# labicon/dp-ilqr

Measured on AMD Instinct MI355X. Metric: ilqr_subproblems_per_sec, higher is better.
Workload: dtype f64; 1 GPU; cfg2: batches of 1024 independent 5-agent DoubleIntDynamics4D iLQR sub-problems per GPU per step, T=50, scripts/analysis.py scenario distribution, tol=1e-3, n_lqr_iter=50; 2468 steps = 2527232 distinct seeds per GPU, window of 6144 in flight; 1 repetition(s) of the job on disjoint seeds, the median is reported; batch_per_gpu=1024, window=6144, n_x=20, n_u=10, horizon=50, parallelism=single GPU

## Files before the change

### dpilqr_amd/csrc/admit_order.hpp

```cpp
#pragma once
#include <cstdint>

#if defined(__HIPCC__)
#include <hip/hip_runtime.h>
#define DPILQR_HD __host__ __device__
#else
#define DPILQR_HD
#endif

namespace dpilqr {

enum CostOrder : int { kOrderOff = 0, kOrderSpread = 1, kOrderGrouped = 2 };
constexpr int kDefaultCostOrder = kOrderSpread;

constexpr int kOrderMinLive = 1024;
constexpr int kOrderClasses = 64;

struct SweepDeal {
    int n, n_cus, waves, per_layer, layers, rounds, lo, extra;
    DPILQR_HD SweepDeal(int n_, int n_cus_, int waves_) : n(n_), n_cus(n_cus_), waves(waves_) {
        const int lpr = waves / 4;
        per_layer = 4 * n_cus;
        layers = (n + per_layer - 1) / per_layer;
        rounds = (layers + lpr - 1) / lpr;
        lo = rounds > 0 ? layers / rounds : 0;
        extra = rounds > 0 ? layers - lo * rounds : 0;
    }
    DPILQR_HD int layers_of(int round) const { return lo + (round < extra ? 1 : 0); }
    DPILQR_HD int first_layer(int round) const { return round * lo + (round < extra ? round : extra); }
    DPILQR_HD int round_of_layer(int layer) const {
        const int head = extra * (lo + 1);
        return layer < head ? layer / (lo + 1) : extra + (layer - head) / (lo > 0 ? lo : 1);
    }
    DPILQR_HD int slot(int round, int cu, int wave) const {
        if (round >= rounds || wave >= 4 * layers_of(round)) return -1;
        const int s = (first_layer(round) + (wave >> 2)) * per_layer + (wave & 3) * n_cus + cu;
        return s < n ? s : -1;
    }
};

DPILQR_HD inline int order_position(int rank, const SweepDeal& D, int order) {
    if (order != kOrderGrouped) return rank;
    const int round = D.round_of_layer(rank / D.per_layer);
    const int f = D.first_layer(round), m = D.layers_of(round);
    const int q = rank - f * D.per_layer;
    int base = 4 * m, e = 0;
    if (round == D.rounds - 1) {
        const int rem = D.n - (D.layers - 1) * D.per_layer;
        base = 4 * (m - 1) + rem / D.n_cus;
        e = rem % D.n_cus;
    }
    int cu, w;
    if (q < e * (base + 1)) { cu = q / (base + 1); w = q - cu * (base + 1); }
    else { const int q2 = q - e * (base + 1), per = base > 0 ? base : 1; cu = e + q2 / per; w = q2 - (cu - e) * per; }
    return (f + (w >> 2)) * D.per_layer + (w & 3) * D.n_cus + cu;
}

DPILQR_HD inline int order_class(int key, int T) {
    const int top = T + 1;
    const int c = top < kOrderClasses ? key : (int)((int64_t)key * (kOrderClasses - 1) / top);
    return c < 0 ? 0 : (c > kOrderClasses - 1 ? kOrderClasses - 1 : c);
}

#if defined(__HIPCC__) && defined(DPILQR_ADMIT_ORDER_KERNELS)

constexpr int kKeyStagedAgents = 5;
__global__ void __launch_bounds__(256) k_cost_keys(const double* __restrict__ X, const double* __restrict__ radius, int64_t radius_bstride,
                                                   const int32_t* __restrict__ list, const int32_t* __restrict__ count, int B, int T, int k,
                                                   int min_live, int32_t* __restrict__ key) {
    __shared__ double2 sP[4][64 * kKeyStagedAgents];
    const int n = count ? *count : B;
    if (n <= min_live) return;
    const int wave = (int)threadIdx.x >> 6, lane = threadIdx.x & 63;
    const int pos = (int)blockIdx.x * 4 + wave;
    if (pos >= n) return;
    const int b = list ? list[pos] : pos;
    if (b < 0 || b >= B) return;
    const double r = radius[(int64_t)b * radius_bstride];
    const double lim = r * r * (1.0 + 1e-12);
    const int nx = 4 * k;
    const double* Xb = X + (int64_t)b * (T + 1) * nx;
    const bool staged = k <= kKeyStagedAgents;
    int cnt = 0;
    for (int t0 = 0; t0 <= T; t0 += 64) {
        const int rows = min(64, T + 1 - t0);
        bool near = false;
        if (staged) {
            const double2* src = reinterpret_cast<const double2*>(Xb + (int64_t)t0 * nx);
            for (int e = lane; e < rows * k; e += 64) sP[wave][e] = src[2 * e];
            __builtin_amdgcn_wave_barrier();
            asm volatile("" ::: "memory");
            if (lane < rows) {
                double2 p[kKeyStagedAgents];
#pragma unroll
                for (int i = 0; i < kKeyStagedAgents; ++i) p[i] = sP[wave][lane * k + min(i, k - 1)];
#pragma unroll
                for (int i = 0; i < kKeyStagedAgents; ++i)
#pragma unroll
                    for (int j = i + 1; j < kKeyStagedAgents; ++j) {
                        const double ddx = p[i].x - p[j].x, ddy = p[i].y - p[j].y;
                        const double s2 = ddx * ddx + ddy * ddy;
                        near = near || (j < k && !(s2 > lim));
                    }
            }
            __builtin_amdgcn_wave_barrier();
            asm volatile("" ::: "memory");
        } else if (lane < rows) {
            const double* row = Xb + (int64_t)(t0 + lane) * nx;
            for (int i = 0; i < k; ++i)
                for (int j = i + 1; j < k; ++j) {
                    const double ddx = row[4 * i] - row[4 * j], ddy = row[4 * i + 1] - row[4 * j + 1];
                    const double s2 = ddx * ddx + ddy * ddy;
                    near = near || !(s2 > lim);
                }
        }
        cnt += __popcll(__builtin_amdgcn_ballot_w64(near));
    }
    if (lane == 0) key[pos] = cnt;
}

__global__ void __launch_bounds__(1024) k_order_list(const int32_t* __restrict__ src, int32_t* __restrict__ dst, const int32_t* __restrict__ count,
                                                     const int32_t* __restrict__ key, int T, int n_cus, int waves, int order, int min_live) {
    static_assert(kOrderClasses == 64, "the prefix sums below are one wavefront's, a bin per lane");
    __shared__ int hist[kOrderClasses], cursor[kOrderClasses];
    const int n = *count;
    if (n <= min_live || order == kOrderOff) {
        for (int i = threadIdx.x; i < n; i += blockDim.x) dst[i] = src[i];
        return;
    }
    if (threadIdx.x < kOrderClasses) hist[threadIdx.x] = 0;
    __syncthreads();
    for (int i = threadIdx.x; i < n; i += blockDim.x) atomicAdd(&hist[kOrderClasses - 1 - order_class(key[i], T)], 1);
    __syncthreads();
    if (threadIdx.x < kOrderClasses) {
        const int own = hist[threadIdx.x];
        int run = own;
        for (int off = 1; off < kOrderClasses; off <<= 1) {
            const int below = __shfl_up(run, off);
            if ((int)threadIdx.x >= off) run += below;
        }
        cursor[threadIdx.x] = run - own;
    }
    __syncthreads();
    const SweepDeal deal(n, n_cus, waves);
    for (int i = threadIdx.x; i < n; i += blockDim.x) {
        const int rank = atomicAdd(&cursor[kOrderClasses - 1 - order_class(key[i], T)], 1);
        const int pos = order_position(rank, deal, order);
        if (pos >= 0 && pos < n) dst[pos] = src[i];
    }
}

#endif

}
```

### dpilqr_amd/csrc/dpilqr_hip.hip

```cpp
#include <hip/hip_runtime.h>

#include <cstdarg>
#include <cstdio>
#include <algorithm>
#include <cstdlib>
#include <cstring>
#include <new>
#include <vector>

#include "dpilqr_hip.h"
#include "admit_order.hpp"
#include "launch.hpp"
#include "models.hpp"
#include "tiles.hpp"

namespace dpilqr {

static thread_local char g_err[512] = "";

int32_t fail(int32_t code, const char* fmt, ...) {
    va_list ap;
    va_start(ap, fmt);
    vsnprintf(g_err, sizeof(g_err), fmt, ap);
    va_end(ap);
    return code;
}
const char* last_error() { return g_err; }

const char* route_env(const char* name) {
    static const bool open = [] { const char* g = std::getenv("DPILQR_DEBUG_ROUTES"); return g && g[0] == '1' && g[1] == 0; }();
    return open ? std::getenv(name) : nullptr;
}

int device_cus() {
    static int cus_of[64] = {0};
    int dev = 0;
    if (hipGetDevice(&dev) != hipSuccess || dev < 0 || dev >= 64) return 256;
    if (cus_of[dev] == 0) {
        int n = 0;
        if (hipDeviceGetAttribute(&n, hipDeviceAttributeMultiprocessorCount, dev) != hipSuccess || n <= 0) n = 256;
        cus_of[dev] = n;
    }
    return cus_of[dev];
}

}

using namespace dpilqr;

namespace {

constexpr int kMaxAgents = 64;

int family_nc(int ns) { return ns == 3 ? 2 : ns == 4 ? 2 : ns == 5 ? 2 : ns == 6 ? 3 : ns == 12 ? 4 : -1; }

int32_t check_family5(const dpilqr_batch_desc* d, bool f32) {
    if (d->n_s != 5) return DPILQR_OK;
    if (f32) return fail(DPILQR_EUNSUPPORTED, "the fp32 arm does not serve the five-state family (BikeDynamics5D)");
    if (d->k * d->n_s > 60)
        return fail(DPILQR_EUNSUPPORTED, "k=%d BikeDynamics5D agents (n_x=%d): the five-state family is served up to 12 agents (n_x <= 60)",
                    d->k, d->k * d->n_s);
    return DPILQR_OK;
}

int32_t check_desc(const dpilqr_batch_desc* d, int max_k = kMaxAgents) {
    if (!d) return fail(DPILQR_EINVAL, "desc is NULL");
    if (d->B < 0 || d->k < 1 || d->T < 1) return fail(DPILQR_EINVAL, "bad sizes B=%d k=%d T=%d", d->B, d->k, d->T);
    if (d->k > max_k) return fail(DPILQR_EUNSUPPORTED, "k=%d agents per sub-problem exceeds %d", d->k, max_k);
    if (family_nc(d->n_s) != d->n_c)
        return fail(DPILQR_EINVAL, "(n_s,n_c)=(%d,%d) is not a model family; expected (3,2),(4,2),(5,2),(6,3),(12,4)", d->n_s, d->n_c);
    if (d->B > 0 && (!d->model || !d->n_dims || !d->xf || !d->Q || !d->R || !d->Qf || !d->radius))
        return fail(DPILQR_EINVAL, "desc holds a NULL device pointer");
    const uintptr_t ints = reinterpret_cast<uintptr_t>(d->model) | reinterpret_cast<uintptr_t>(d->n_dims);
    const uintptr_t dbls = reinterpret_cast<uintptr_t>(d->xf) | reinterpret_cast<uintptr_t>(d->Q) | reinterpret_cast<uintptr_t>(d->R) |
                           reinterpret_cast<uintptr_t>(d->Qf) | reinterpret_cast<uintptr_t>(d->radius);
    if (d->B > 0 && (ints % alignof(int32_t) != 0 || dbls % alignof(double) != 0))
        return fail(DPILQR_EINVAL, "desc holds a device pointer that is not aligned to its element type");
    return check_family5(d, false);
}

hipStream_t as_stream(void* s) { return reinterpret_cast<hipStream_t>(s); }

void alpha_table(double* a) {
    static const uint32_t bits[DPILQR_N_ALPHA] = {0x3f800000u, 0x3f68ba2eu, 0x3f2ed9f7u, 0x3ed92350u, 0x3e5eda27u,
                                                  0x3dbd05a8u, 0x3d04808du, 0x3c19864au, 0x3b13029cu, 0x39e8ae70u};
    for (int i = 0; i < DPILQR_N_ALPHA; ++i) {
        float f;
        memcpy(&f, &bits[i], 4);
        a[i] = (double)f;
    }
}

__global__ void k_init_state(int B, double* mu, double* delta, int32_t* status, int32_t* n_bwd, int32_t* n_fwd,
                             int32_t* singular, int32_t* counts, int n_counts, double* alphas_dev, double a0, double a1,
                             double a2, double a3, double a4, double a5, double a6, double a7, double a8, double a9) {
    const int i = blockIdx.x * blockDim.x + threadIdx.x;
    if (i < B) {
        mu[i] = 1.0; delta[i] = 2.0; status[i] = DPILQR_STATUS_ACTIVE; n_bwd[i] = 0; n_fwd[i] = 0; singular[i] = 0;
    }
    if (i < n_counts) counts[i] = 0;
    if (i == 0) {
        alphas_dev[0] = a0; alphas_dev[1] = a1; alphas_dev[2] = a2; alphas_dev[3] = a3; alphas_dev[4] = a4;
        alphas_dev[5] = a5; alphas_dev[6] = a6; alphas_dev[7] = a7; alphas_dev[8] = a8; alphas_dev[9] = a9;
    }
}

__global__ void k_admit(int32_t* list, int32_t* count, int32_t* next_count, int32_t* admitted, int B, int window,
                        int32_t* mail, int want_prefix, int64_t* t_admit, const int32_t* fault) {
    const int base = *count, first = *admitted;
    const int n_new = min(B - first, window - base);
    __shared__ int lowest;
    if (threadIdx.x == 0) lowest = first;
    __syncthreads();
    for (int i = threadIdx.x; i < n_new; i += blockDim.x) list[base + i] = first + i;
    if (t_admit && n_new > 0) {
        const int64_t now = (int64_t)__builtin_amdgcn_s_memrealtime();
        for (int i = threadIdx.x; i < n_new; i += blockDim.x) t_admit[first + i] = now;
    }
    if (mail && want_prefix) {
        int lo = first;
        for (int i = threadIdx.x; i < base; i += blockDim.x) lo = min(lo, list[i]);
        for (int off = 32; off > 0; off >>= 1) lo = min(lo, __shfl_down(lo, off));
        if ((threadIdx.x & 63) == 0) atomicMin(&lowest, lo);
        __syncthreads();
    }
    if (threadIdx.x == 0) {
        *count = base + n_new; *admitted = first + n_new; *next_count = 0;
        if (mail) { mail[0] = base + n_new; mail[1] = first + n_new; mail[2] = want_prefix ? lowest : 0; mail[3] = *fault; }
    }
}

__global__ void k_copy_f64(int n, const double* src, double* dst) {
    const int i = blockIdx.x * blockDim.x + threadIdx.x;
    if (i < n) dst[i] = src[i];
}

__global__ void k_finish_status(int B, int32_t* status) {
    const int i = blockIdx.x * blockDim.x + threadIdx.x;
    if (i < B && status[i] == DPILQR_STATUS_ACTIVE) status[i] = DPILQR_STATUS_MAX_ITER;
}

constexpr int kCountRing = 4;

struct SolveShape {
    bool big;
    size_t elem;
    bool fused;
};

struct SolveWorkspace {
    size_t tiles, K, d, Xc, Uc, mu, delta, J_star, J_last, alphas, singular, lists, counts, t_admit, total;
    SolveWorkspace(const dpilqr_batch_desc& D, int W, bool gains_in_ws, SolveShape sh) {
        const size_t B = D.B, n = (size_t)D.k * D.n_s, m = (size_t)D.k * D.n_c, T = D.T, Wn = W, e = sh.elem;
        const TileLayout L((int)n, (int)m);
        auto al = [](size_t x) { return (x + 255) & ~(size_t)255; };
        size_t o = 0;
        tiles = o;    o = al(o + (sh.big ? e * Wn * (size_t)riccati_big_scratch_elems((int)n, (int)m)
                                         : (sh.fused ? 0 : sizeof(double) * Wn * (T + 1) * L.stride)));
        K = o;        o = al(o + (gains_in_ws ? e * Wn * T * m * n : 0));
        d = o;        o = al(o + (gains_in_ws ? e * Wn * T * m : 0));
        Xc = o;       o = al(o + e * Wn * DPILQR_N_ALPHA * (T + 1) * n);
        Uc = o;       o = al(o + e * Wn * DPILQR_N_ALPHA * T * m);
        mu = o;       o = al(o + sizeof(double) * B);
        delta = o;    o = al(o + sizeof(double) * B);
        J_star = o;   o = al(o + sizeof(double) * B);
        J_last = o;   o = al(o + sizeof(double) * B);
        alphas = o;   o = al(o + sizeof(double) * DPILQR_N_ALPHA);
        singular = o; o = al(o + sizeof(int32_t) * B);
        lists = o;    o = al(o + sizeof(int32_t) * 2 * Wn);
        counts = o;   o = al(o + sizeof(int32_t) * (kCountRing + 2));
        t_admit = o;  o = al(o + sizeof(int64_t) * B);
        total = o;
    }
};
constexpr int kMaxLqrIter = 4096;
constexpr int kMaxGlobalIter = 1 << 20;

int window_of(const dpilqr_batch_desc& D, int window) { return (window <= 0 || window > D.B) ? (D.B > 0 ? D.B : 1) : window; }

constexpr int kHostLag = 3, kMailRing = kHostLag + 1, kMailWords = 4;

struct Profiler {
    bool on = false;
    int mask = 0xF;
    bool skip = false;
    double ms[4] = {0, 0, 0, 0};
    int64_t launches[4] = {0, 0, 0, 0}, items[4] = {0, 0, 0, 0};
    double sweep_ms[3] = {0, 0, 0};
    int64_t sweep_launches[3] = {0, 0, 0}, sweep_items[3] = {0, 0, 0};
    std::vector<hipEvent_t> pool;
    struct Rec { int cls, iter; size_t e0; int tag; };
    std::vector<Rec> recs;
    size_t used = 0;
    ~Profiler() {
        for (auto& e : pool) (void)hipEventDestroy(e);
    }
    hipEvent_t next() {
        if (used == pool.size()) {
            hipEvent_t e;
            if (hipEventCreate(&e) != hipSuccess) return nullptr;
            pool.push_back(e);
        }
        return pool[used++];
    }
    void begin(int cls, int iter, hipStream_t st) {
        skip = !on || !((mask >> cls) & 1);
        if (skip) return;
        recs.push_back({cls, iter, used, 0});
        hipEvent_t e = next();
        if (e) (void)hipEventRecord(e, st);
    }
    void end(hipStream_t st, int tag = 0) {
        if (skip) return;
        hipEvent_t e = next();
        if (e) (void)hipEventRecord(e, st);
        recs.back().tag = tag;
    }
    void drop() { recs.clear(); used = 0; }
    void collect(const std::vector<int32_t>& active, int B) {
        if (!on) { drop(); return; }
        for (const Rec& r : recs) {
            float t = 0.f;
            if (r.e0 + 1 < pool.size() && hipEventElapsedTime(&t, pool[r.e0], pool[r.e0 + 1]) == hipSuccess) {
                const int64_t n_it = (r.iter < 0) ? B : (r.iter < (int)active.size() ? active[r.iter] : 0);
                ms[r.cls] += t;
                launches[r.cls] += 1;
                items[r.cls] += n_it;
                if (r.cls == 1 && (r.tag == 4 || r.tag == 8 || r.tag == 12)) {
                    const int v = r.tag / 4 - 1;
                    sweep_ms[v] += t; sweep_launches[v] += 1; sweep_items[v] += n_it;
                }
            }
        }
        drop();
    }
};

}

struct dpilqr_solver {
    int device = -1;
    int32_t* host = nullptr;
    int32_t* dev = nullptr;
    std::vector<int32_t> hist;
    hipEvent_t ev[kMailRing] = {};
    Profiler prof;
    dpilqr_progress_fn progress = nullptr;
    void* progress_user = nullptr;
    int32_t init() {
        HIP_TRY(hipGetDevice(&device));
        HIP_TRY(hipHostMalloc(reinterpret_cast<void**>(&host), sizeof(int32_t) * kMailWords * kMailRing, hipHostMallocDefault));
        HIP_TRY(hipHostGetDevicePointer(reinterpret_cast<void**>(&dev), host, 0));
        for (auto& e : ev) HIP_TRY(hipEventCreateWithFlags(&e, hipEventDisableTiming));
        return DPILQR_OK;
    }
    void release() {
        if (host) (void)hipHostFree(host);
        host = nullptr;
        for (auto& e : ev) {
            if (e) (void)hipEventDestroy(e);
            e = nullptr;
        }
    }
    ~dpilqr_solver() { release(); }
};

namespace {

thread_local dpilqr_solver g_default_solver;

int32_t default_solver(dpilqr_solver** out) {
    int dev = 0;
    HIP_TRY(hipGetDevice(&dev));
    if (g_default_solver.host && g_default_solver.device != dev) g_default_solver.release();
    if (!g_default_solver.host) {
        int32_t rc = g_default_solver.init();
        if (rc) return rc;
    }
    *out = &g_default_solver;
    return DPILQR_OK;
}

__global__ void k_normalise_lists(int32_t* lists, int32_t* counts, int window, int it_end, int src) {
    const int cs = it_end % kCountRing;
    __shared__ int n_sh;
    if (threadIdx.x == 0) n_sh = counts[cs];
    __syncthreads();
    const int n = n_sh;
    if (src == 1)
        for (int i = threadIdx.x; i < n; i += blockDim.x) lists[i] = lists[window + i];
    __syncthreads();
    if (threadIdx.x == 0) {
        for (int c = 0; c < kCountRing; ++c) counts[c] = 0;
        counts[0] = n;
    }
}

template <typename R> struct Passes;
template <> struct Passes<double> {
    static int32_t forward(const dpilqr_batch_desc& D, int mode, const double* x0, double* X, double* U, const double* K,
                           const double* d, const double* alphas, int ngrp, double* Xc, double* Uc, double* Jc,
                           const SolveState& S, const int32_t* items, const int32_t* n_items, int grid, hipStream_t st) {
        return launch_forward(D, mode, x0, X, U, K, d, alphas, ngrp, Xc, Uc, Jc, S, items, n_items, grid, st);
    }
    static int32_t sweep_big(const dpilqr_batch_desc& D, const double* X, const double* U, const double* mu, double* K, double* d,
                             int32_t* sing, const int32_t* items, const int32_t* n_items, int grid, int by_item, void* scratch,
                             hipStream_t st) {
        return launch_riccati_big_f64(D, X, U, mu, K, d, sing, items, n_items, grid, by_item, scratch, st);
    }
};
template <> struct Passes<float> {
    static int32_t forward(const dpilqr_batch_desc& D, int mode, const float* x0, float* X, float* U, const float* K,
                           const float* d, const double* alphas, int ngrp, float* Xc, float* Uc, double* Jc,
                           const SolveState& S, const int32_t* items, const int32_t* n_items, int grid, hipStream_t st) {
        return launch_forward_big_f32(D, mode, x0, X, U, K, d, alphas, ngrp, Xc, Uc, Jc, S, items, n_items, grid, st);
    }
    static int32_t sweep_big(const dpilqr_batch_desc& D, const float* X, const float* U, const double* mu, float* K, float* d,
                             int32_t* sing, const int32_t* items, const int32_t* n_items, int grid, int by_item, void* scratch,
                             hipStream_t st) {
        return launch_riccati_big_f32(D, X, U, mu, K, d, sing, items, n_items, grid, by_item, scratch, st);
    }
};

template <typename R>
SolveShape shape_of(const dpilqr_batch_desc& D) {
    const bool big = sizeof(R) == 4 || uses_big_path(D.k * D.n_s);
    return SolveShape{big, sizeof(R), !big && fused_sweep_applies(D) && !solve_prefers_records(D)};
}

template <typename R>
int32_t solve_impl(dpilqr_solver* solver, const dpilqr_batch_desc* desc, const R* x0, R* U, int32_t n_lqr_iter, double tol,
                   double t_kill, int32_t window, void* workspace, int64_t workspace_bytes, R* X, double* J, int32_t* status,
                   int32_t* n_bwd, int32_t* n_fwd, double* trace, R* K_out, R* d_out, int32_t n_global_iter,
                   int32_t resume, hipStream_t st) {
    int32_t rc = check_desc(desc);
    if (!rc) rc = check_family5(desc, sizeof(R) == 4);
    if (rc) return rc;
    if (desc->B == 0) return DPILQR_OK;
    if (!x0 || !U || !X || !J || !status || !n_bwd || !n_fwd || !workspace)
        return fail(DPILQR_EINVAL, "solve_batch: NULL pointer");
    if ((K_out == nullptr) != (d_out == nullptr)) return fail(DPILQR_EINVAL, "solve_batch: K_out and d_out go together");
    if (n_lqr_iter < 0 || n_lqr_iter > kMaxLqrIter) return fail(DPILQR_EINVAL, "solve_batch: n_lqr_iter=%d", n_lqr_iter);
    if (!solver && n_global_iter < 0) return fail(DPILQR_EINVAL, "solve_enqueue: n_global_iter=%d", n_global_iter);
    const dpilqr_batch_desc& D = *desc;
    const int Wn = window_of(D, window);
    const bool gains_by_item = K_out != nullptr;
    const SolveShape sh = shape_of<R>(D);
    const SolveWorkspace W(D, Wn, !gains_by_item, sh);
    if (workspace_bytes < (int64_t)W.total)
        return fail(DPILQR_EWORKSPACE, "solve_batch: workspace %lld B < required %zu B", (long long)workspace_bytes, W.total);
    if (solver) {
        int dev = 0;
        HIP_TRY(hipGetDevice(&dev));
        if (dev != solver->device)
            return fail(DPILQR_EINVAL, "solve_batch: the solver belongs to device %d, the current device is %d", solver->device, dev);
    }
    char* ws = static_cast<char*>(workspace);
    double* tiles = reinterpret_cast<double*>(ws + W.tiles);
    R* K = gains_by_item ? K_out : reinterpret_cast<R*>(ws + W.K);
    R* d = gains_by_item ? d_out : reinterpret_cast<R*>(ws + W.d);
    double* alphas = reinterpret_cast<double*>(ws + W.alphas);
    R* Xc = reinterpret_cast<R*>(ws + W.Xc);
    R* Uc = reinterpret_cast<R*>(ws + W.Uc);
    int32_t* lists = reinterpret_cast<int32_t*>(ws + W.lists);
    int32_t* counts = reinterpret_cast<int32_t*>(ws + W.counts);
    int32_t* singular = reinterpret_cast<int32_t*>(ws + W.singular);
    SolveState S{};
    S.mu = reinterpret_cast<double*>(ws + W.mu);
    S.delta = reinterpret_cast<double*>(ws + W.delta);
    S.J_star = reinterpret_cast<double*>(ws + W.J_star);
    S.J_last = reinterpret_cast<double*>(ws + W.J_last);
    S.status = status; S.n_bwd = n_bwd; S.n_fwd = n_fwd; S.trace = trace; S.singular = singular;
    S.n_lqr_iter = n_lqr_iter; S.tol = tol; S.gains_by_item = gains_by_item ? 1 : 0;
    int64_t* t_admit = nullptr;
    S.t_admit = nullptr; S.t_kill_ticks = 0;
    if (t_kill > 0.0) {
        int dev_now = 0, khz = 0;
        HIP_TRY(hipGetDevice(&dev_now));
        if (hipDeviceGetAttribute(&khz, hipDeviceAttributeWallClockRate, dev_now) != hipSuccess || khz <= 0) khz = 100000;
        const double ticks = t_kill * 1e3 * (double)khz;
        S.t_kill_ticks = ticks < 1.0 ? 1 : (ticks > 9e18 ? (int64_t)9e18 : (int64_t)ticks);
        t_admit = reinterpret_cast<int64_t*>(ws + W.t_admit);
        S.t_admit = t_admit;
    }
    const int n = D.k * D.n_s, m = D.k * D.n_c;
    Profiler none;
    Profiler& prof = solver ? solver->prof : none;
    if (solver) solver->hist.clear();
    auto bail = [&](int32_t code) {
        (void)hipStreamSynchronize(st);
        prof.drop();
        return code;
    };

    int32_t* admitted_dev = counts + kCountRing;
    S.fault = counts + kCountRing + 1;
    static const bool no_static = route_flag("DPILQR_TILES_NO_STATIC");
    const int um = hint_model(D);
    const bool fused = sh.fused;
    const bool static_part = !fused && !sh.big && !no_static && D.R_bstride == 0 &&
                             (um == kDoubleInt4D || um == kDoubleInt6D || um == kHumanLin6D);
    if (!resume) {
        double a[DPILQR_N_ALPHA];
        alpha_table(a);
        const int init_n = D.B > kCountRing + 2 ? D.B : kCountRing + 2;
        hipLaunchKernelGGL(k_init_state, dim3((init_n + 255) / 256), dim3(256), 0, st, D.B, S.mu, S.delta, status, n_bwd, n_fwd,
                           singular, counts, kCountRing + 2, alphas, a[0], a[1], a[2], a[3], a[4], a[5], a[6], a[7], a[8], a[9]);
        HIP_TRY(hipGetLastError());
        prof.begin(3, -1, st);
        rc = Passes<R>::forward(D, kModeRollout, x0, X, U, nullptr, nullptr, nullptr, 1, nullptr, nullptr, S.J_star, S, nullptr,
                                nullptr, D.B, st);
        if (rc) return bail(rc);
        prof.end(st);
        hipLaunchKernelGGL(k_copy_f64, dim3((D.B + 255) / 256), dim3(256), 0, st, D.B, S.J_star, S.J_last);
        if (n_lqr_iter > 0) {
            if (!fused && hipMemsetAsync(tiles, 0, W.K - W.tiles, st) != hipSuccess) return bail(fail(DPILQR_EHIP, "hipMemsetAsync failed"));
            if (static_part) {
                if constexpr (sizeof(R) == 8) {
                    if ((rc = launch_make_tiles(D, X, U, tiles, nullptr, nullptr, Wn, true, false, st))) return bail(rc);
                }
            }
        }
    }

    static const int order_route = route_flag("DPILQR_NO_COST_ORDER") ? (int)kOrderOff : route_int("DPILQR_COST_ORDER", kDefaultCostOrder);
    const int order = (sizeof(R) == 8 && fused && (order_route == kOrderSpread || order_route == kOrderGrouped)) ? order_route : (int)kOrderOff;
    int32_t* keys = reinterpret_cast<int32_t*>(ws + W.Xc);
    int surv = 0;
    size_t n_iterations = 0;
    auto enqueue_iteration = [&](int it, int upper) -> int32_t {
        int32_t* cur = lists + (size_t)surv * Wn;
        int32_t* other = lists + (size_t)(surv ^ 1) * Wn;
        int32_t* cur_n = counts + (it % kCountRing);
        int32_t* nxt_n = counts + ((it + 1) % kCountRing);
        int32_t* mail = solver ? solver->dev + kMailWords * (it % kMailRing) : nullptr;
        hipLaunchKernelGGL(k_admit, dim3(1), dim3(256), 0, st, cur, cur_n, nxt_n, admitted_dev, D.B, Wn, mail,
                           (solver && solver->progress) ? 1 : 0, t_admit, S.fault);
        if (solver) HIP_TRY(hipEventRecord(solver->ev[it % kMailRing], st));
        int32_t r = DPILQR_OK;
        const int order_waves = order ? fused_sweep_tier(D, upper) : 0;
        if (order_waves > 0) {
            if constexpr (sizeof(R) == 8) {
                if ((r = launch_cost_keys(D, X, cur, cur_n, upper, kOrderMinLive, keys, st))) return r;
                if ((r = launch_order_list(cur, other, cur_n, keys, D.T, device_cus(), order_waves, order, kOrderMinLive, st))) return r;
            }
            S.next_items = cur;
            cur = other;
        } else {
            S.next_items = other;
            surv ^= 1;
        }
        S.next_count = nxt_n;
        if (fused) {
            if constexpr (sizeof(R) == 8) {
                prof.begin(1, it, st);
                if ((r = launch_riccati_fused(D, X, U, S.mu, K, d, singular, cur, cur_n, upper, S.gains_by_item, st))) return r;
                prof.end(st, g_sweep_waves);
            }
        } else if (!sh.big) {
            if constexpr (sizeof(R) == 8) {
                prof.begin(0, it, st);
                if ((r = launch_make_tiles(D, X, U, tiles, cur, cur_n, upper, true, static_part, st))) return r;
                prof.end(st);
                prof.begin(1, it, st);
                if ((r = launch_riccati(D.B, D.T, n, m, tiles, S.mu, K, d, singular, cur, cur_n, upper, S.gains_by_item, D.n_s,
                                        D.n_c, st)))
                    return r;
                prof.end(st, g_sweep_waves);
            }
        } else {
            prof.begin(1, it, st);
            if ((r = Passes<R>::sweep_big(D, X, U, S.mu, K, d, singular, cur, cur_n, upper, S.gains_by_item, tiles, st))) return r;
            prof.end(st, 0);
        }
        prof.begin(2, it, st);
        if ((r = Passes<R>::forward(D, kModeLineSearch, nullptr, X, U, K, d, alphas, DPILQR_N_ALPHA, Xc, Uc, nullptr, S, cur, cur_n,
                                    upper, st)))
            return r;
        prof.end(st);
        return DPILQR_OK;
    };

    if (n_lqr_iter > 0 && solver) {
        int upper = Wn;
        int32_t reported = 0;
        for (int it = 0; it < kMaxGlobalIter; ++it) {
            n_iterations = (size_t)it + 1;
            if ((rc = enqueue_iteration(it, upper))) return bail(rc);
            bool done = false;
            if (it >= kHostLag) {
                const int slot = (it - kHostLag) % kMailRing;
                if (hipEventSynchronize(solver->ev[slot]) != hipSuccess) return bail(fail(DPILQR_EHIP, "hipEventSynchronize failed"));
                const int32_t act = solver->host[kMailWords * slot], adm = solver->host[kMailWords * slot + 1];
                const int32_t prefix = solver->host[kMailWords * slot + 2];
                solver->hist.push_back(act);
                if (solver->progress && prefix > reported) { reported = prefix; solver->progress(solver->progress_user, prefix, D.B); }
                done = (adm >= D.B && act == 0);
                upper = (adm >= D.B) ? std::min(Wn, std::max(act, 1)) : Wn;
            }
            if (done) break;
            if (it + 1 == kMaxGlobalIter) return bail(fail(DPILQR_EUNSUPPORTED, "solve_batch: more than %d global iterations", kMaxGlobalIter));
        }
    } else if (n_lqr_iter > 0) {
        for (int it = 0; it < n_global_iter; ++it)
            if ((rc = enqueue_iteration(it, Wn))) return rc;
        if (n_global_iter > 0)
            hipLaunchKernelGGL(k_normalise_lists, dim3(1), dim3(256), 0, st, lists, counts, Wn, n_global_iter, surv);
    }
    hipLaunchKernelGGL(k_copy_f64, dim3((D.B + 255) / 256), dim3(256), 0, st, D.B, S.J_last, J);
    if (n_lqr_iter == 0) hipLaunchKernelGGL(k_finish_status, dim3((D.B + 255) / 256), dim3(256), 0, st, D.B, status);
    HIP_TRY(hipGetLastError());
    if (!solver) return DPILQR_OK;
    if (hipStreamSynchronize(st) != hipSuccess) return bail(fail(DPILQR_EHIP, "hipStreamSynchronize failed"));
    if (n_lqr_iter > 0) {
        for (size_t j = solver->hist.size(); j < n_iterations; ++j) solver->hist.push_back(solver->host[kMailWords * (j % kMailRing)]);
    }
    prof.collect(solver->hist, D.B);
    if (solver->progress) solver->progress(solver->progress_user, D.B, D.B);
    if (n_lqr_iter > 0) {
        int32_t faulted = 0;
        for (int j = 0; j < kMailRing; ++j) faulted = std::max(faulted, solver->host[kMailWords * j + 3]);
        if (faulted > 0)
            return fail(DPILQR_EHIP, "solve_batch: the device gave up %d of %d items (status DPILQR_STATUS_FAULT: a hand-over inside a "
                                     "team of workgroups expired); every other item's result is valid", faulted, D.B);
    }
    return DPILQR_OK;
}

}

extern "C" {

int32_t dpilqr_abi_version(void) { return DPILQR_ABI_VERSION; }
const char* dpilqr_last_error(void) { return last_error(); }

int32_t dpilqr_device_info(int32_t dev, int32_t* n_cu, int32_t* lds_bytes, char* arch, int32_t arch_len) {
    int count = 0;
    if (hipGetDeviceCount(&count) != hipSuccess || count <= 0) return fail(DPILQR_ENOGPU, "no HIP device visible");
    if (dev < 0 || dev >= count) return fail(DPILQR_EINVAL, "device %d out of range (%d visible)", dev, count);
    hipDeviceProp_t p;
    HIP_TRY(hipGetDeviceProperties(&p, dev));
    if (n_cu) *n_cu = p.multiProcessorCount;
    if (lds_bytes) *lds_bytes = (int32_t)p.maxSharedMemoryPerMultiProcessor;
    if (arch && arch_len > 0) { strncpy(arch, p.gcnArchName, arch_len - 1); arch[arch_len - 1] = 0; }
    if (strncmp(p.gcnArchName, "gfx950", 6) != 0)
        return fail(DPILQR_ENOGPU, "device %d is %s; this library is built for gfx950 only", dev, p.gcnArchName);
    return DPILQR_OK;
}

int32_t dpilqr_model_dims(int32_t model, int32_t* n_s, int32_t* n_c) {
    if (model < 0 || model >= kNumModels || model_ns(model) < 0 || !n_s || !n_c) return fail(DPILQR_EINVAL, "unknown model %d", model);
    *n_s = model_ns(model);
    *n_c = model_nc(model);
    return DPILQR_OK;
}

static int32_t model_op(int op, int32_t n, int32_t ns, const int32_t* model, const double* x, const double* u, double dt,
                        double* o1, double* o2, void* stream) {
    if (n < 0 || !model || !x || !u || !o1 || (op == 2 && !o2)) return fail(DPILQR_EINVAL, "model op: bad argument");
    if (n == 0) return DPILQR_OK;
    return launch_model_op(op, n, ns, model, x, u, dt, o1, o2, as_stream(stream));
}

int32_t dpilqr_model_f(int32_t n, int32_t family_ns, const int32_t* model, const double* x, const double* u,
                       double* x_dot, void* stream) {
    return model_op(0, n, family_ns, model, x, u, 0.0, x_dot, nullptr, stream);
}
int32_t dpilqr_model_integrate(int32_t n, int32_t family_ns, const int32_t* model, const double* x, const double* u,
                               double dt, double* x_new, void* stream) {
    return model_op(1, n, family_ns, model, x, u, dt, x_new, nullptr, stream);
}
int32_t dpilqr_model_linearize(int32_t n, int32_t family_ns, const int32_t* model, const double* x, const double* u,
                               double dt, double* A, double* B, void* stream) {
    return model_op(2, n, family_ns, model, x, u, dt, A, B, stream);
}

int32_t dpilqr_cost_eval(const dpilqr_batch_desc* desc, int32_t n_pts, const double* x, const double* u,
                         int32_t terminal, double* cost, void* stream) {
    int32_t rc = check_desc(desc);
    if (rc) return rc;
    if (n_pts < 0 || !x || !u || !cost) return fail(DPILQR_EINVAL, "cost_eval: bad argument");
    if ((int64_t)desc->B * n_pts == 0) return DPILQR_OK;
    return launch_cost_eval(*desc, n_pts, x, u, terminal, cost, as_stream(stream));
}

int32_t dpilqr_tile_layout(int32_t n_x, int32_t n_u, int64_t offsets[7], int64_t row_strides[7], int64_t* stride) {
    if (n_x < 1 || n_u < 1 || !offsets || !row_strides || !stride) return fail(DPILQR_EINVAL, "tile_layout: bad argument");
    return tile_layout_host(n_x, n_u, offsets, row_strides, stride);
}

int64_t dpilqr_tiles_bytes(int32_t B, int32_t T, int32_t n_x, int32_t n_u) {
    if (B < 0 || T < 1 || n_x < 1 || n_u < 1) return fail(DPILQR_EINVAL, "tiles_bytes: bad argument");
    return (int64_t)sizeof(double) * B * (T + 1) * TileLayout(n_x, n_u).stride;
}

int32_t dpilqr_make_tiles(const dpilqr_batch_desc* desc, const double* X, const double* U, double* tiles,
                          const int32_t* items, const int32_t* n_items, void* stream) {
    int32_t rc = check_desc(desc);
    if (rc) return rc;
    if (!X || !U || !tiles) return fail(DPILQR_EINVAL, "make_tiles: NULL pointer");
    return launch_make_tiles(*desc, X, U, tiles, items, n_items, desc->B, false, false, as_stream(stream));
}

int32_t dpilqr_rollout(const dpilqr_batch_desc* desc, const double* x0, const double* U, double* X, double* J,
                       void* stream) {
    int32_t rc = check_desc(desc);
    if (rc) return rc;
    if (desc->B == 0) return DPILQR_OK;
    if (!x0 || !U || !X || !J) return fail(DPILQR_EINVAL, "rollout: NULL pointer");
    SolveState S{};
    return launch_forward(*desc, kModeRollout, x0, X, const_cast<double*>(U), nullptr, nullptr, nullptr, 1, nullptr,
                          nullptr, J, S, nullptr, nullptr, desc->B, as_stream(stream));
}

int32_t dpilqr_rollout_wide(const dpilqr_batch_desc* desc, const double* x0, const double* U, double* X, double* J,
                            double* min_sep, double* goal_dist, void* stream) {
    const int32_t rc = check_desc(desc, 256);
    if (rc) return rc;
    if (!x0 || !U || !J) return fail(DPILQR_EINVAL, "rollout_wide: NULL pointer");
    uintptr_t dbls = 0;
    for (const double* p : {x0, U, (const double*)X, (const double*)J, (const double*)min_sep, (const double*)goal_dist}) dbls |= reinterpret_cast<uintptr_t>(p);
    if (dbls % alignof(double) != 0) return fail(DPILQR_EINVAL, "rollout_wide: a device pointer is not aligned to its element type");
    return launch_rollout_wide(*desc, x0, U, X, J, min_sep, goal_dist, as_stream(stream));
}

int32_t dpilqr_backward_pass_tiles(int32_t B, int32_t T, int32_t n_x, int32_t n_u, const double* tiles,
                                   const double* mu, double* K, double* d, int32_t* singular, const int32_t* items,
                                   const int32_t* n_items, void* stream) {
    if (B < 0 || T < 1 || n_x < 1 || n_u < 1) return fail(DPILQR_EINVAL, "backward_pass_tiles: bad sizes");
    if (!tiles || !mu || !K || !d) return fail(DPILQR_EINVAL, "backward_pass_tiles: NULL pointer");
    return launch_riccati(B, T, n_x, n_u, tiles, mu, K, d, singular, items, n_items, B, 0, 0, 0, as_stream(stream));
}

int32_t dpilqr_backward_pass_tiles_blocks(int32_t B, int32_t T, int32_t n_x, int32_t n_u, int32_t block_ns,
                                          int32_t block_nc, const double* tiles, const double* mu, double* K,
                                          double* d, int32_t* singular, const int32_t* items,
                                          const int32_t* n_items, void* stream) {
    if (B < 0 || T < 1 || n_x < 1 || n_u < 1) return fail(DPILQR_EINVAL, "backward_pass_tiles_blocks: bad sizes");
    if (!tiles || !mu || !K || !d) return fail(DPILQR_EINVAL, "backward_pass_tiles_blocks: NULL pointer");
    if (block_ns < 0 || block_nc < 0 || (block_ns > 0 && (block_nc < 1 || n_x % block_ns || n_u % block_nc ||
                                                          n_x / block_ns != n_u / block_nc)))
        return fail(DPILQR_EINVAL, "backward_pass_tiles_blocks: n_x=%d, n_u=%d are not k blocks of %d, %d", n_x, n_u,
                    block_ns, block_nc);
    return launch_riccati(B, T, n_x, n_u, tiles, mu, K, d, singular, items, n_items, B, 0, block_ns, block_nc,
                          as_stream(stream));
}

int64_t dpilqr_backward_pass_workspace_bytes(const dpilqr_batch_desc* desc, int32_t elem_bytes) {
    if (!desc || desc->B < 0 || desc->k < 1 || desc->T < 1 || (elem_bytes != 4 && elem_bytes != 8))
        return fail(DPILQR_EINVAL, "backward_pass_workspace_bytes: bad argument");
    const int n = desc->k * desc->n_s, m = desc->k * desc->n_c;
    if (elem_bytes == 4 || uses_big_path(n)) return (int64_t)elem_bytes * desc->B * riccati_big_scratch_elems(n, m);
    return (int64_t)sizeof(double) * desc->B * (desc->T + 1) * TileLayout(n, m).stride;
}

int32_t dpilqr_backward_pass(const dpilqr_batch_desc* desc, const double* X, const double* U, const double* mu,
                             double* K, double* d, double* tiles_workspace, void* stream) {
    int32_t rc = check_desc(desc);
    if (rc) return rc;
    if (desc->B == 0) return DPILQR_OK;
    if (!X || !U || !mu || !K || !d || !tiles_workspace) return fail(DPILQR_EINVAL, "backward_pass: NULL pointer");
    const int n = desc->k * desc->n_s, m = desc->k * desc->n_c;
    if (uses_big_path(n)) {
        HIP_TRY(hipMemsetAsync(tiles_workspace, 0, sizeof(double) * desc->B * (size_t)riccati_big_scratch_elems(n, m), as_stream(stream)));
        return launch_riccati_big_f64(*desc, X, U, mu, K, d, nullptr, nullptr, nullptr, desc->B, 0, tiles_workspace, as_stream(stream));
    }
    rc = launch_make_tiles(*desc, X, U, tiles_workspace, nullptr, nullptr, desc->B, false, false, as_stream(stream));
    if (rc) return rc;
    return launch_riccati(desc->B, desc->T, n, m, tiles_workspace, mu, K, d, nullptr, nullptr, nullptr, desc->B, 0, desc->n_s,
                          desc->n_c, as_stream(stream));
}

int32_t dpilqr_backward_pass_fused(const dpilqr_batch_desc* desc, const double* X, const double* U, const double* mu, double* K,
                                   double* d, int32_t* singular, void* stream) {
    int32_t rc = check_desc(desc);
    if (rc) return rc;
    if (desc->B == 0) return DPILQR_OK;
    if (!X || !U || !mu || !K || !d) return fail(DPILQR_EINVAL, "backward_pass_fused: NULL pointer");
    if (!fused_sweep_applies(*desc))
        return fail(DPILQR_EUNSUPPORTED, "backward_pass_fused: needs 6..15 four-state, 1..10 six-state, 1..6 CarDynamics3D or 1..4 BikeDynamics5D agents, or at most five "
                                         "DoubleIntDynamics4D / UnicycleDynamics4D agents with n_dims = 2 (uniform_model hints)");
    rc = launch_riccati_fused(*desc, X, U, mu, K, d, singular, nullptr, nullptr, desc->B, 0, as_stream(stream));
    return rc == DPILQR_EUNSUPPORTED ? fail(rc, "backward_pass_fused: no instantiation for n_x=%d", desc->k * desc->n_s) : rc;
}

int32_t dpilqr_backward_pass_f32(const dpilqr_batch_desc* desc, const float* X, const float* U, const double* mu, float* K,
                                 float* d, void* workspace, void* stream) {
    int32_t rc = check_desc(desc);
    if (!rc) rc = check_family5(desc, true);
    if (rc) return rc;
    if (desc->B == 0) return DPILQR_OK;
    if (!X || !U || !mu || !K || !d || !workspace) return fail(DPILQR_EINVAL, "backward_pass_f32: NULL pointer");
    const int n = desc->k * desc->n_s, m = desc->k * desc->n_c;
    HIP_TRY(hipMemsetAsync(workspace, 0, sizeof(float) * desc->B * (size_t)riccati_big_scratch_elems(n, m), as_stream(stream)));
    return launch_riccati_big_f32(*desc, X, U, mu, K, d, nullptr, nullptr, nullptr, desc->B, 0, workspace, as_stream(stream));
}

int32_t dpilqr_rollout_f32(const dpilqr_batch_desc* desc, const float* x0, const float* U, float* X, double* J, void* stream) {
    int32_t rc = check_desc(desc);
    if (!rc) rc = check_family5(desc, true);
    if (rc) return rc;
    if (desc->B == 0) return DPILQR_OK;
    if (!x0 || !U || !X || !J) return fail(DPILQR_EINVAL, "rollout_f32: NULL pointer");
    SolveState S{};
    return launch_forward_big_f32(*desc, kModeRollout, x0, X, const_cast<float*>(U), nullptr, nullptr, nullptr, 1, nullptr, nullptr,
                                  J, S, nullptr, nullptr, desc->B, as_stream(stream));
}

int32_t dpilqr_forward_pass_f32(const dpilqr_batch_desc* desc, const float* X, const float* U, const float* K, const float* d,
                                const double* alphas, int32_t n_alpha, float* Xn, float* Un, double* Jn, void* stream) {
    int32_t rc = check_desc(desc);
    if (!rc) rc = check_family5(desc, true);
    if (rc) return rc;
    if (desc->B == 0) return DPILQR_OK;
    if (!X || !U || !K || !d || !alphas || !Xn || !Un || !Jn) return fail(DPILQR_EINVAL, "forward_pass_f32: NULL pointer");
    if (n_alpha < 1) return fail(DPILQR_EINVAL, "forward_pass_f32: n_alpha=%d", n_alpha);
    SolveState S{};
    return launch_forward_big_f32(*desc, kModeCandidates, nullptr, const_cast<float*>(X), const_cast<float*>(U), K, d, alphas,
                                  n_alpha, Xn, Un, Jn, S, nullptr, nullptr, desc->B, as_stream(stream));
}

int32_t dpilqr_forward_pass(const dpilqr_batch_desc* desc, const double* X, const double* U, const double* K,
                            const double* d, const double* alphas, int32_t n_alpha, double* Xn, double* Un, double* Jn,
                            void* stream) {
    int32_t rc = check_desc(desc);
    if (rc) return rc;
    if (!X || !U || !K || !d || !alphas || !Xn || !Un || !Jn) return fail(DPILQR_EINVAL, "forward_pass: NULL pointer");
    if (n_alpha < 1) return fail(DPILQR_EINVAL, "forward_pass: n_alpha=%d", n_alpha);
    SolveState S{};
    return launch_forward(*desc, kModeCandidates, nullptr, const_cast<double*>(X), const_cast<double*>(U), K, d, alphas,
                          n_alpha, Xn, Un, Jn, S, nullptr, nullptr, desc->B, as_stream(stream));
}

static int32_t check_policy_args(const char* who, const dpilqr_batch_desc* desc, int32_t n_samples, const double* X, const double* U,
                                 const double* K, const double* x0s, const double* J, const double* W, const double* u_lim,
                                 const double* Xs, const double* Us, const double* min_sep, const double* goal_dist) {
    const int32_t rc = check_desc(desc);
    if (rc) return rc;
    if (!X || !U || !K || !x0s || !J) return fail(DPILQR_EINVAL, "%s: NULL pointer", who);
    if (n_samples <= 0) return fail(DPILQR_EINVAL, "%s: n_samples=%d", who, n_samples);
    uintptr_t dbls = 0;
    for (const double* p : {X, U, K, x0s, J, W, u_lim, Xs, Us, min_sep, goal_dist}) dbls |= reinterpret_cast<uintptr_t>(p);
    return dbls % alignof(double) == 0 ? DPILQR_OK : fail(DPILQR_EINVAL, "%s: a device pointer is not aligned to its element type", who);
}

int32_t dpilqr_policy_rollout(const dpilqr_batch_desc* desc, const double* X, const double* U, const double* K, int32_t n_samples,
                              const double* x0s, const double* W, const double* u_lim, double* Xs, double* Us, double* J,
                              double* min_sep, double* goal_dist, void* stream) {
    const int32_t rc = check_policy_args("policy_rollout", desc, n_samples, X, U, K, x0s, J, W, u_lim, Xs, Us, min_sep, goal_dist);
    return rc ? rc : launch_policy_rollout(*desc, X, U, K, n_samples, x0s, W, u_lim, Xs, Us, J, min_sep, goal_dist, as_stream(stream));
}

int32_t dpilqr_policy_rollout_large(const dpilqr_batch_desc* desc, const double* X, const double* U, const double* K, int32_t n_samples,
                                    const double* x0s, const double* W, const double* u_lim, double* Xs, double* Us, double* J,
                                    double* min_sep, double* goal_dist, void* stream) {
    const int32_t rc = check_policy_args("policy_rollout_large", desc, n_samples, X, U, K, x0s, J, W, u_lim, Xs, Us, min_sep, goal_dist);
    return rc ? rc : launch_policy_rollout_large(*desc, X, U, K, n_samples, x0s, W, u_lim, Xs, Us, J, min_sep, goal_dist, as_stream(stream));
}

int32_t dpilqr_policy_rollout_dec(const dpilqr_batch_desc* desc, const double* X, const double* U_ff, const double* Kc, int32_t kc_max,
                                  const uint64_t* nbr_bits, int32_t n_samples, const double* x0s, const double* W, const double* u_lim,
                                  double* Xs, double* Us, double* J, double* min_sep, double* goal_dist, void* stream) {
    const int32_t rc = check_policy_args("policy_rollout_dec", desc, n_samples, X, U_ff, Kc, x0s, J, W, u_lim, Xs, Us, min_sep, goal_dist);
    if (rc) return rc;
    if (!nbr_bits || reinterpret_cast<uintptr_t>(nbr_bits) % alignof(uint64_t) != 0)
        return fail(DPILQR_EINVAL, "policy_rollout_dec: nbr_bits is a NULL pointer or not aligned to its element type");
    return launch_policy_rollout_dec(*desc, X, U_ff, Kc, kc_max, nbr_bits, n_samples, x0s, W, u_lim, Xs, Us, J, min_sep, goal_dist,
                                     as_stream(stream));
}

static int32_t check_advance_args(const char* who, const dpilqr_batch_desc* desc, const double* X, const double* U, const double* K,
                                  int32_t h, const int32_t* scen, int32_t n_scen, int32_t L, int32_t n_d, const double* W,
                                  const double* u_lim, const double* x_cur, const int32_t* n_done, const double* X_exec,
                                  const double* U_exec, const double* J_exec, const double* min_sep, const double* dist_left,
                                  const double* U_next, const double* X_next) {
    const int32_t rc = check_desc(desc);
    if (rc) return rc;
    if (!X || !U || !x_cur || !n_done || !X_exec || !U_exec || !J_exec || !min_sep || !dist_left || !U_next || !X_next)
        return fail(DPILQR_EINVAL, "%s: NULL pointer", who);
    if (h < 1 || h > desc->T) return fail(DPILQR_EINVAL, "%s: h=%d, a round executes 1 .. T = %d steps", who, h, desc->T);
    if (L < 1) return fail(DPILQR_EINVAL, "%s: L=%d", who, L);
    if (n_d < 1 || n_d > desc->n_s) return fail(DPILQR_EINVAL, "%s: n_d=%d, an agent has n_s = %d states", who, n_d, desc->n_s);
    if (n_scen < desc->B) return fail(DPILQR_EINVAL, "%s: n_scen=%d for B = %d items", who, n_scen, desc->B);
    uintptr_t dbls = 0;
    for (const double* p : {X, U, K, W, u_lim, x_cur, X_exec, U_exec, J_exec, min_sep, dist_left, U_next, X_next}) dbls |= reinterpret_cast<uintptr_t>(p);
    const uintptr_t ints = reinterpret_cast<uintptr_t>(scen) | reinterpret_cast<uintptr_t>(n_done);
    return dbls % alignof(double) == 0 && ints % alignof(int32_t) == 0
               ? DPILQR_OK : fail(DPILQR_EINVAL, "%s: a device pointer is not aligned to its element type", who);
}

int32_t dpilqr_policy_advance(const dpilqr_batch_desc* desc, const double* X, const double* U, const double* K, int32_t h,
                              const int32_t* scen, int32_t n_scen, int32_t L, int32_t n_d, const double* W, const double* u_lim,
                              double* x_cur, int32_t* n_done, double* X_exec, double* U_exec, double* J_exec, double* min_sep,
                              double* dist_left, double* U_next, double* X_next, void* stream) {
    const int32_t rc = check_advance_args("policy_advance", desc, X, U, K, h, scen, n_scen, L, n_d, W, u_lim, x_cur, n_done, X_exec,
                                          U_exec, J_exec, min_sep, dist_left, U_next, X_next);
    return rc ? rc : launch_policy_advance(*desc, X, U, K, 0, nullptr, h, scen, n_scen, L, n_d, W, u_lim, x_cur, n_done, X_exec, U_exec,
                                           J_exec, min_sep, dist_left, U_next, X_next, as_stream(stream));
}

int32_t dpilqr_policy_advance_large(const dpilqr_batch_desc* desc, const double* X, const double* U, const double* K, int32_t h,
                                    const int32_t* scen, int32_t n_scen, int32_t L, int32_t n_d, const double* W, const double* u_lim,
                                    double* x_cur, int32_t* n_done, double* X_exec, double* U_exec, double* J_exec, double* min_sep,
                                    double* dist_left, double* U_next, double* X_next, void* stream) {
    int32_t rc = check_advance_args("policy_advance_large", desc, X, U, K, h, scen, n_scen, L, n_d, W, u_lim, x_cur, n_done,
                                    X_exec, U_exec, J_exec, min_sep, dist_left, U_next, X_next);
    if (rc == DPILQR_EUNSUPPORTED && desc->n_s == 5)
        rc = fail(DPILQR_EUNSUPPORTED, "policy_advance_large: the (5, 2) family is served up to n_x = 60, by dpilqr_policy_advance; "
                                       "served here are the (4, 2), (6, 3) and (12, 4) families with 60 < n_x <= 240, k <= 20");
    return rc ? rc : launch_policy_advance_large(*desc, X, U, K, h, scen, n_scen, L, n_d, W, u_lim, x_cur, n_done, X_exec, U_exec,
                                                 J_exec, min_sep, dist_left, U_next, X_next, as_stream(stream));
}

int32_t dpilqr_policy_advance_dec(const dpilqr_batch_desc* desc, const double* X, const double* U_ff, const double* Kc,
                                  int32_t kc_max, const uint64_t* nbr_bits, int32_t h, const int32_t* scen, int32_t n_scen,
                                  int32_t L, int32_t n_d, const double* W, const double* u_lim, double* x_cur, int32_t* n_done,
                                  double* X_exec, double* U_exec, double* J_exec, double* min_sep, double* dist_left,
                                  double* U_next, double* X_next, void* stream) {
    const int32_t rc = check_advance_args("policy_advance_dec", desc, X, U_ff, Kc, h, scen, n_scen, L, n_d, W, u_lim, x_cur, n_done,
                                          X_exec, U_exec, J_exec, min_sep, dist_left, U_next, X_next);
    if (rc) return rc;
    if ((Kc && !nbr_bits) || reinterpret_cast<uintptr_t>(nbr_bits) % alignof(uint64_t) != 0)
        return fail(DPILQR_EINVAL, "policy_advance_dec: nbr_bits is a NULL pointer or not aligned to its element type");
    if (kc_max < 1 || kc_max > desc->k)
        return fail(DPILQR_EUNSUPPORTED, "policy_advance_dec: kc_max=%d, a neighbourhood has 1 .. k = %d members", kc_max, desc->k);
    return launch_policy_advance(*desc, X, U_ff, Kc, kc_max, nbr_bits, h, scen, n_scen, L, n_d, W, u_lim, x_cur, n_done, X_exec, U_exec,
                                 J_exec, min_sep, dist_left, U_next, X_next, as_stream(stream));
}

int32_t dpilqr_alphas(double* alphas_host) {
    if (!alphas_host) return fail(DPILQR_EINVAL, "alphas: NULL pointer");
    alpha_table(alphas_host);
    return DPILQR_OK;
}

int64_t dpilqr_solve_workspace_bytes(const dpilqr_batch_desc* desc, int32_t window, int32_t gains_in_workspace) {
    if (!desc || desc->B < 0 || desc->k < 1 || desc->T < 1) return fail(DPILQR_EINVAL, "solve_workspace_bytes: bad desc");
    return (int64_t)SolveWorkspace(*desc, window_of(*desc, window), gains_in_workspace != 0, shape_of<double>(*desc)).total;
}
int64_t dpilqr_solve_workspace_bytes_f32(const dpilqr_batch_desc* desc, int32_t window, int32_t gains_in_workspace) {
    if (!desc || desc->B < 0 || desc->k < 1 || desc->T < 1) return fail(DPILQR_EINVAL, "solve_workspace_bytes_f32: bad desc");
    return (int64_t)SolveWorkspace(*desc, window_of(*desc, window), gains_in_workspace != 0, shape_of<float>(*desc)).total;
}

int32_t dpilqr_solver_create(dpilqr_solver** out) {
    if (!out) return fail(DPILQR_EINVAL, "solver_create: NULL pointer");
    dpilqr_solver* s = new (std::nothrow) dpilqr_solver();
    if (!s) return fail(DPILQR_EHIP, "solver_create: out of host memory");
    const int32_t rc = s->init();
    if (rc) { delete s; return rc; }
    *out = s;
    return DPILQR_OK;
}
int32_t dpilqr_solver_destroy(dpilqr_solver* solver) {
    delete solver;
    return DPILQR_OK;
}
int32_t dpilqr_solver_set_progress(dpilqr_solver* solver, dpilqr_progress_fn fn, void* user) {
    if (!solver) {
        const int32_t rc = default_solver(&solver);
        if (rc) return rc;
    }
    solver->progress = fn;
    solver->progress_user = user;
    return DPILQR_OK;
}

int32_t dpilqr_solve_batch(dpilqr_solver* solver, const dpilqr_batch_desc* desc, const double* x0, double* U,
                           int32_t n_lqr_iter, double tol, double t_kill, int32_t window, void* workspace, int64_t workspace_bytes,
                           double* X, double* J, int32_t* status, int32_t* n_bwd, int32_t* n_fwd, double* trace,
                           double* K_out, double* d_out, void* stream) {
    if (!solver) {
        const int32_t rc = default_solver(&solver);
        if (rc) return rc;
    }
    return solve_impl<double>(solver, desc, x0, U, n_lqr_iter, tol, t_kill, window, workspace, workspace_bytes, X, J, status, n_bwd,
                              n_fwd, trace, K_out, d_out, 0, 0, as_stream(stream));
}
int32_t dpilqr_solve_batch_f32(dpilqr_solver* solver, const dpilqr_batch_desc* desc, const float* x0, float* U,
                               int32_t n_lqr_iter, double tol, double t_kill, int32_t window, void* workspace, int64_t workspace_bytes,
                               float* X, double* J, int32_t* status, int32_t* n_bwd, int32_t* n_fwd, double* trace,
                               float* K_out, float* d_out, void* stream) {
    if (!solver) {
        const int32_t rc = default_solver(&solver);
        if (rc) return rc;
    }
    return solve_impl<float>(solver, desc, x0, U, n_lqr_iter, tol, t_kill, window, workspace, workspace_bytes, X, J, status, n_bwd,
                             n_fwd, trace, K_out, d_out, 0, 0, as_stream(stream));
}
int32_t dpilqr_solve_enqueue(const dpilqr_batch_desc* desc, const double* x0, double* U, int32_t n_lqr_iter, double tol,
                             double t_kill, int32_t window, void* workspace, int64_t workspace_bytes, double* X, double* J, int32_t* status,
                             int32_t* n_bwd, int32_t* n_fwd, double* trace, double* K_out, double* d_out,
                             int32_t n_global_iter, int32_t resume, void* stream) {
    return solve_impl<double>(nullptr, desc, x0, U, n_lqr_iter, tol, t_kill, window, workspace, workspace_bytes, X, J, status, n_bwd,
                              n_fwd, trace, K_out, d_out, n_global_iter, resume, as_stream(stream));
}
int64_t dpilqr_solve_iterations_bound(const dpilqr_batch_desc* desc, int32_t window, int32_t n_lqr_iter) {
    if (!desc || desc->B < 0 || n_lqr_iter < 0) return fail(DPILQR_EINVAL, "solve_iterations_bound: bad argument");
    const int64_t W = window_of(*desc, window);
    return ((int64_t)desc->B + W - 1) / W * n_lqr_iter + 1;
}

int32_t dpilqr_debug_stamps(void* buf) {
    int32_t rc = set_stamp_buffer_riccati(buf);
    return rc ? rc : set_stamp_buffer_forward(buf);
}

int32_t dpilqr_cost_keys(const dpilqr_batch_desc* desc, const double* X, const int32_t* items, const int32_t* n_items, int32_t* keys,
                         void* stream) {
    int32_t rc = check_desc(desc);
    if (rc) return rc;
    if (desc->n_s != 4) return fail(DPILQR_EUNSUPPORTED, "cost_keys: n_s=%d, the keys are defined for the four-state family", desc->n_s);
    if (desc->B == 0) return DPILQR_OK;
    if (!X || !keys || ((items == nullptr) != (n_items == nullptr))) return fail(DPILQR_EINVAL, "cost_keys: NULL pointer");
    return launch_cost_keys(*desc, X, items, n_items, desc->B, -1, keys, as_stream(stream));
}

int32_t dpilqr_order_list(const int32_t* items, const int32_t* n_items, const int32_t* keys, int32_t T, int32_t n_cus, int32_t waves,
                          int32_t order, int32_t* out, void* stream) {
    if (!items || !n_items || !keys || !out) return fail(DPILQR_EINVAL, "order_list: NULL pointer");
    if (T < 1 || n_cus < 1 || (waves != 4 && waves != 8 && waves != 12) || (order != kOrderSpread && order != kOrderGrouped))
        return fail(DPILQR_EINVAL, "order_list: T=%d n_cus=%d waves=%d order=%d", T, n_cus, waves, order);
    return launch_order_list(items, out, n_items, keys, T, n_cus, waves, order, -1, as_stream(stream));
}

int32_t dpilqr_order_position(int32_t rank, int32_t n, int32_t n_cus, int32_t waves, int32_t order) {
    if (n < 1 || rank < 0 || rank >= n || n_cus < 1 || (waves != 4 && waves != 8 && waves != 12) ||
        (order != kOrderSpread && order != kOrderGrouped))
        return fail(DPILQR_EINVAL, "order_position: rank=%d n=%d n_cus=%d waves=%d order=%d", rank, n, n_cus, waves, order);
    return order_position(rank, SweepDeal(n, n_cus, waves), order);
}

int32_t dpilqr_profile_enable(dpilqr_solver* solver, int32_t enable) {
    Profiler& g_prof = solver ? solver->prof : g_default_solver.prof;
    const int32_t prev = g_prof.on ? 1 : 0;
    g_prof.on = (enable & 1) != 0;
    g_prof.mask = (enable >> 1) & 0xF ? (enable >> 1) & 0xF : 0xF;
    return prev;
}

int32_t dpilqr_profile_read(dpilqr_solver* solver, double ms[4], int64_t launches[4], int64_t items[4], int32_t reset) {
    if (!ms || !launches || !items) return fail(DPILQR_EINVAL, "profile_read: NULL pointer");
    Profiler& g_prof = solver ? solver->prof : g_default_solver.prof;
    for (int c = 0; c < 4; ++c) {
        ms[c] = g_prof.ms[c]; launches[c] = g_prof.launches[c]; items[c] = g_prof.items[c];
        if (reset) { g_prof.ms[c] = 0; g_prof.launches[c] = 0; g_prof.items[c] = 0; }
    }
    return DPILQR_OK;
}

int32_t dpilqr_profile_read_sweep(dpilqr_solver* solver, int32_t waves, double* ms, int64_t* launches, int64_t* items, int32_t reset) {
    if (!ms || !launches || !items) return fail(DPILQR_EINVAL, "profile_read_sweep: NULL pointer");
    if (waves != 4 && waves != 8 && waves != 12) return fail(DPILQR_EINVAL, "profile_read_sweep: waves=%d (4, 8 or 12)", waves);
    const int v = waves / 4 - 1;
    Profiler& g_prof = solver ? solver->prof : g_default_solver.prof;
    *ms = g_prof.sweep_ms[v]; *launches = g_prof.sweep_launches[v]; *items = g_prof.sweep_items[v];
    if (reset) { g_prof.sweep_ms[v] = 0; g_prof.sweep_launches[v] = 0; g_prof.sweep_items[v] = 0; }
    return DPILQR_OK;
}

int32_t dpilqr_pairwise_graph(int32_t S, int32_t N, int32_t k, int32_t n_s, const double* X, const double* radius,
                              int32_t* adj, void* stream) {
    if (S < 0 || N < 1 || k < 1 || n_s < 2 || !X || !radius || !adj) return fail(DPILQR_EINVAL, "pairwise_graph: bad argument");
    if (S == 0) return DPILQR_OK;
    return launch_pairwise_graph(S, N, k, n_s, X, radius, adj, as_stream(stream));
}

}
```

### dpilqr_amd/csrc/forward_wave.hpp

```cpp
#pragma once
#include <hip/hip_runtime.h>

#include "forward.hpp"
#include "wave_util.hpp"

namespace dpilqr {

template <int KA>
struct PairTable {
    int i[KA * (KA - 1) / 2 + 1], j[KA * (KA - 1) / 2 + 1];
    constexpr PairTable() : i{}, j{} {
        int p = 0;
        for (int a = 0; a < KA; ++a)
            for (int b = a + 1; b < KA; ++b) { i[p] = a; j[p] = b; ++p; }
    }
};

__device__ inline int linesearch_decide(const SolveState& S, int b, int ngrp, const double* sJ) {
    const int iter = S.n_bwd[b];
    const double J_star = S.J_star[b];
    int acc = -1;
    for (int i = 0; i < ngrp; ++i)
        if (sJ[i] < J_star) { acc = i; break; }
    const int n_eval = (acc >= 0) ? acc + 1 : ngrp;
    const double J_last = sJ[n_eval - 1];
    const double mu_before = S.mu[b];
    int status = DPILQR_STATUS_ACTIVE;
    double J_new = J_star;
    if (acc >= 0) {
        const bool conv = fabs((J_star - J_last) / J_star) < S.tol;
        J_new = J_last;
        double delta = fmin(1.0, S.delta[b]) / 2.0;
        double mu = mu_before * delta;
        if (mu <= 1e-6) mu = 0.0;
        S.delta[b] = delta; S.mu[b] = mu; S.J_star[b] = J_new;
        if (conv) status = DPILQR_STATUS_CONVERGED;
        else if (solve_time_is_up(S, b)) status = DPILQR_STATUS_KILLED;
        else if (iter + 1 >= S.n_lqr_iter) status = DPILQR_STATUS_MAX_ITER;
    } else {
        status = DPILQR_STATUS_LINESEARCH_FAILED;
    }
    S.J_last[b] = J_last;
    S.n_fwd[b] += n_eval;
    S.n_bwd[b] = iter + 1;
    S.status[b] = status;
    if (S.trace) {
        double* tr = S.trace + ((int64_t)b * S.n_lqr_iter + iter) * 5;
        tr[0] = mu_before; tr[1] = (double)acc; tr[2] = J_last; tr[3] = J_new; tr[4] = (double)n_eval;
    }
    if (status == DPILQR_STATUS_ACTIVE && S.next_items) {
        const int pos = atomicAdd(S.next_count, 1);
        S.next_items[pos] = b;
    }
    return acc;
}

template <int NS>
__device__ __forceinline__ double pair_cost_nd(const double* a, const double* b, int nd, double radius) {
    const double dx = a[0] - b[0], dy = a[1] - b[1];
    double s = 0.0;
    s += dx * dx;
    s += dy * dy;
    if (NS >= 3) {
        const double dz = a[2] - b[2];
        const double s3 = s + dz * dz;
        s = (nd >= 3) ? s3 : s;
    }
    if (nd < 2) s = dx * dx;
    if (s > radius * radius * (1.0 + 1e-12)) return 0.0;
    const double m = fmin(0.0, sqrt(s) - radius);
    return m * m;
}

template <int MODEL, int KA>
struct WaveFwdLds {
    static constexpr int NS = ModelDef<MODEL>::NS, NC = ModelDef<MODEL>::NC;
    static constexpr int n = KA * NS, m = KA * NC, NP = KA * (KA - 1) / 2, NP1 = NP > 0 ? NP : 1;
    static constexpr int LDG = (n % 4 == 0) ? n + 2 : n;
    static constexpr int NW = (KA * DPILQR_N_ALPHA + 63) / 64;
#ifndef DPILQR_LS_KGAP_ALL
#define DPILQR_LS_KGAP_ALL 0
#endif
#ifndef DPILQR_LS_NO_KGAP
#define DPILQR_LS_NO_KGAP 0
#endif
    static constexpr int kgap_for(int blk) { int g = 0; while ((((blk + g) / 2) & 1) == 0) g += 2; return g; }
    static constexpr int KBLK = NC * n;
    static constexpr int KGAP = (!DPILQR_LS_NO_KGAP && (NW > 1 || DPILQR_LS_KGAP_ALL) && KBLK % 2 == 0) ? kgap_for(KBLK) : 0;
    static constexpr int oK = 0;
    static constexpr int od = oK + m * n + KA * KGAP;
    static constexpr int odx = (od + m + 1) & ~1;
    static constexpr int oxs = odx + DPILQR_N_ALPHA * LDG;
    static constexpr int ocr = oxs + DPILQR_N_ALPHA * LDG;
    static constexpr int ocp = ocr + 2 * DPILQR_N_ALPHA * KA;
    static constexpr int oJ = ocp + 2 * DPILQR_N_ALPHA * NP1;
    static constexpr int IPB = NW == 1 ? 4 : 1;
    static constexpr int octl = oJ + DPILQR_N_ALPHA;
#ifndef DPILQR_LS_CL_ALL
#define DPILQR_LS_CL_ALL 0
#endif
    static constexpr bool CONST_LDS = NW > 1 || NS >= 6 || DPILQR_LS_CL_ALL;
#ifndef DPILQR_LS_OCC
#define DPILQR_LS_OCC 2
#endif
    static constexpr int OCC = ((NW > 1 && NS >= 6 && KA >= 9) || NS >= 12) ? 1 : DPILQR_LS_OCC;
#ifndef DPILQR_LS_PF
#define DPILQR_LS_PF 2
#endif
    static constexpr int PF = (NW == 1 && NS == 4 && !CONST_LDS) ? DPILQR_LS_PF : 1;
    static_assert(PF == 1 || PF == 2, "the horizon loop is written out for one or two register stages (step t, step t + 1)");
    static constexpr int oQ = (octl + 2 + 1) & ~1;
    static constexpr int oR = oQ + (CONST_LDS ? KA * NS * NS : 0);
    static constexpr int oXf = oR + (CONST_LDS ? KA * NC * NC : 0);
    static constexpr int total = (oXf + (CONST_LDS ? n : 0) + 1) & ~1;
};

template <int NW>
__device__ __forceinline__ void wave_sync() {
    if constexpr (NW == 1) asm volatile("" ::: "memory");
    else asm volatile("s_waitcnt lgkmcnt(0)\n\ts_barrier" ::: "memory");
}

template <int MODEL, int KA>
__global__ __launch_bounds__((64 * WaveFwdLds<MODEL, KA>::NW * WaveFwdLds<MODEL, KA>::IPB), (WaveFwdLds<MODEL, KA>::OCC)) void k_linesearch_wave(
    dpilqr_batch_desc D, double* X, double* U, const double* __restrict__ K, const double* __restrict__ d,
    const double* __restrict__ alphas, double* Xc, double* Uc, SolveState S, const int32_t* __restrict__ items,
    const int32_t* __restrict__ n_items) {
    using W = WaveFwdLds<MODEL, KA>;
    constexpr int NS = W::NS, NC = W::NC, n = W::n, m = W::m, mn = m * n, NPAIRS = W::NP, NP1 = W::NP1;
    constexpr int NG = DPILQR_N_ALPHA;
    constexpr int NW = W::NW, NTH = 64 * NW;
    constexpr int PPL = (NPAIRS + KA - 1) / KA;
    constexpr int KV = (mn / 2 + NTH - 1) / NTH;

    const int sub = NW == 1 ? __builtin_amdgcn_readfirstlane((int)(threadIdx.x >> 6)) : 0;
    const int tid = NW == 1 ? (int)(threadIdx.x & 63) : (int)threadIdx.x;
    const int slot = blockIdx.x * W::IPB + sub;
    if (slot >= *n_items) return;
    const int b = items[slot];
    const int T = D.T;
    extern __shared__ __attribute__((aligned(16))) double lds_all[];
    double* lds = lds_all + sub * W::total;
    double* Xb = X + (int64_t)b * (T + 1) * n;
    double* Ub = U + (int64_t)b * T * m;
    if (S.singular && S.singular[b]) {
        if (tid == 0) retire_without_gains(S, b);
        return;
    }
    const int64_t gslot = S.gains_by_item ? b : slot;
    const double* Kb = K + gslot * T * mn;
    const double* db = d + gslot * T * m;
    const bool active = tid < KA * NG;
    const int g = active ? tid / KA : 0, a = active ? tid - (tid / KA) * KA : 0;
    const double alpha = alphas[g];
    double* const Xw0 = Xc + (int64_t)slot * NG * (int64_t)(T + 1) * n;
    double* const Uw0 = Uc + (int64_t)slot * NG * (int64_t)T * m;
    int xw_off = g * (T + 1) * n + a * NS;
    asm volatile("" : "+v"(xw_off));
    auto uw_off_at = [&](int t_) {
        int g_ = g;
        asm volatile("" : "+v"(g_));
        return (unsigned)(g_ * (T * m) + a * NC + t_ * m);
    };

    const ItemParams P = item_params(D, b);
    constexpr bool CL = W::CONST_LDS;
    double xf_r[CL ? 1 : NS], Q_r[CL ? 1 : NS * NS], R_r[CL ? 1 : NC * NC];
    const double* xf = xf_r; const double* Q = Q_r; const double* R = R_r;
    if constexpr (CL) {
        for (int e = tid; e < KA * NS * NS; e += NTH) lds[W::oQ + e] = P.Q[e];
        for (int e = tid; e < KA * NC * NC; e += NTH) lds[W::oR + e] = P.R[e];
        for (int e = tid; e < n; e += NTH) lds[W::oXf + e] = P.xf[e];
        xf = lds + W::oXf + a * NS; Q = lds + W::oQ + a * NS * NS; R = lds + W::oR + a * NC * NC;
    } else {
#pragma unroll
        for (int i = 0; i < NS; ++i) xf_r[i] = P.xf[a * NS + i];
#pragma unroll
        for (int i = 0; i < NS * NS; ++i) Q_r[i] = P.Q[a * NS * NS + i];
#pragma unroll
        for (int i = 0; i < NC * NC; ++i) R_r[i] = P.R[a * NC * NC + i];
    }
    const double radius = P.radius;
    bool homog = true;
#pragma unroll
    for (int i = 1; i < KA; ++i) homog = homog && (P.n_dims[i] == P.n_dims[0]);
    int pp[PPL > 0 ? PPL : 1];
    auto make_pairs = [&](int a_) {
#pragma unroll
        for (int q = 0; q < PPL; ++q) {
            const int p = min(a_ + q * KA, NP1 - 1);
            int ii = 0, rem = p;
            while (rem >= KA - 1 - ii) { rem -= KA - 1 - ii; ++ii; }
            const int jj = ii + 1 + rem;
            pp[q] = ii | (jj << 8) | ((homog ? 2 : min(P.n_dims[ii], P.n_dims[jj])) << 16);
        }
    };
    make_pairs(a);

    double* sK = lds + W::oK;
    double* sd = lds + W::od;
    double* sdx = lds + W::odx + g * W::LDG;
    double* sxs = lds + W::oxs + g * W::LDG;
    double* scr0 = lds + W::ocr + g * KA;
    double* scp0 = lds + W::ocp + g * NP1;

    struct Stage { v2d stK[KV]; double std_, u[NC], xold[NS]; };
    constexpr int PF = W::PF;
    Stage stg[PF];
    double x[NS];
    auto fetch = [&](Stage& sg, int t) {
        const unsigned ko = (unsigned)(t * mn), xo = (unsigned)(t * n + a * NS), uo = (unsigned)(t * m + a * NC);
#ifdef DPILQR_LS_K_FIRST
#pragma unroll
        for (int q = 0; q < KV; ++q) {
            const int e = min(tid + NTH * q, mn / 2 - 1);
            sg.stK[q] = *reinterpret_cast<const v2d*>(Kb + (ko + 2u * (unsigned)e));
        }
#endif
#pragma unroll
        for (int i = 0; i < NS; ++i) sg.xold[i] = Xb[xo + (unsigned)i];
#pragma unroll
        for (int i = 0; i < NC; ++i) sg.u[i] = Ub[uo + (unsigned)i];
        sg.std_ = db[(unsigned)(t * m + min(tid, m - 1))];
#ifndef DPILQR_LS_K_FIRST
#pragma unroll
        for (int q = 0; q < KV; ++q) {
            const int e = min(tid + NTH * q, mn / 2 - 1);
            sg.stK[q] = *reinterpret_cast<const v2d*>(Kb + (ko + 2u * (unsigned)e));
        }
#endif
    };
    auto store_vec = [&](double* p, const double* v, int len) {
        if ((len & 1) == 0) {
#pragma unroll
            for (int i = 0; i < len; i += 2) store_v2d_nt(p + i, v2d{v[i], v[i + 1]});
        } else {
#pragma unroll
            for (int i = 0; i < len; ++i) store_f64_nt(p + i, v[i]);
        }
    };
    auto stage_cost = [&](double& J, int par) {
        const double* scp = scp0 + par * NG * NP1;
        const double* scr = scr0 + par * NG * KA;
        double prox = 0.0, ref = 0.0;
        if constexpr (NPAIRS > 32) {
            constexpr int CH = 8;
#pragma unroll 1
            for (int p0 = 0; p0 < NPAIRS; p0 += CH) {
                double v[CH];
#pragma unroll
                for (int q = 0; q < CH; ++q) v[q] = scp[min(p0 + q, NP1 - 1)];
#pragma unroll
                for (int q = 0; q < CH; ++q) prox = (p0 + q < NPAIRS) ? prox + v[q] : prox;
            }
        } else {
#pragma unroll
            for (int p = 0; p < NPAIRS; ++p) prox += scp[p];
        }
#pragma unroll
        for (int i = 0; i < KA; ++i) ref += scr[i];
        J += D.w_prox * prox + D.w_ref * ref;
    };
    auto post_costs = [&](double cr, const double* cp, int par) {
        if (active) {
            scr0[par * NG * KA + a] = cr;
#pragma unroll
            for (int q = 0; q < PPL; ++q)
                if (a + q * KA < NPAIRS) scp0[par * NG * NP1 + a + q * KA] = cp[q];
        }
    };

#pragma unroll
    for (int i = 0; i < NS; ++i) x[i] = Xb[a * NS + i];
#pragma unroll
    for (int s = 0; s < PF; ++s)
        if (s < T) fetch(stg[s], s);
    double J = 0.0;
    double ut[NC];
#pragma unroll
    for (int i = 0; i < NC; ++i) ut[i] = 0.0;

#ifdef DPILQR_PHASE_STAMPS
    unsigned long long w_wait = 0, w_t0 = __builtin_amdgcn_s_memtime();
#endif
    auto step = [&](Stage& sg, int t) {
        v2d (&stK)[KV] = sg.stK;
        double& std_ = sg.std_;
        double (&u)[NC] = sg.u;
        double (&xold)[NS] = sg.xold;
#ifdef DPILQR_PHASE_STAMPS
        {
            const unsigned long long a0 = __builtin_amdgcn_s_memtime();
            asm volatile("s_waitcnt vmcnt(0)" ::: "memory");
            w_wait += __builtin_amdgcn_s_memtime() - a0;
        }
#endif
#pragma unroll
        for (int q = 0; q < KV; ++q) {
            int tid_o = tid;
            if constexpr (W::KGAP > 0) asm volatile("" : "+v"(tid_o));
            const int e = min(tid_o + NTH * q, mn / 2 - 1);
            *reinterpret_cast<v2d*>(sK + 2 * e + (W::KGAP > 0 ? ((2 * e) / W::KBLK) * W::KGAP : 0)) = stK[q];
        }
        if (tid < m) sd[tid] = std_;
        if (active) {
            store_vec(Xw0 + (unsigned)(xw_off + t * n), x, NS);
            if (t > 0) store_vec(Uw0 + uw_off_at(t - 1), ut, NC);
        }
#pragma unroll
        for (int i = 0; i < NC; ++i) ut[i] = u[i];
        if (active) {
#pragma unroll
            for (int i = 0; i < NS; ++i) {
                sdx[a * NS + i] = x[i] - xold[i];
                sxs[a * NS + i] = x[i];
            }
        }
        wave_sync<NW>();
        if (t + PF < T) fetch(sg, t + PF);
        if (a == 0 && t > 0) stage_cost(J, (t & 1) ^ 1);
        DPILQR_LDS_FENCE();
        {
            double sum[NC];
#pragma unroll
            for (int c = 0; c < NC; ++c) sum[c] = 0.0;
            const double* rows = sK + a * (W::KBLK + W::KGAP);
            if (n % 2 == 0) {
#pragma unroll 5
                for (int j = 0; j < n; j += 2) {
                    const v2d dx2 = *reinterpret_cast<const v2d*>(lds + W::odx + g * W::LDG + j);
#pragma unroll
                    for (int c = 0; c < NC; ++c) {
                        const v2d kr = *reinterpret_cast<const v2d*>(rows + c * n + j);
                        sum[c] += kr.x * dx2.x;
                        sum[c] += kr.y * dx2.y;
                    }
                }
            } else {
#pragma unroll
                for (int j = 0; j < n; ++j) {
                    const double dxj = lds[W::odx + g * W::LDG + j];
#pragma unroll
                    for (int c = 0; c < NC; ++c) sum[c] += rows[c * n + j] * dxj;
                }
            }
#pragma unroll
            for (int c = 0; c < NC; ++c) {
                const double du = sum[c] + alpha * sd[a * NC + c];
                ut[c] = ut[c] + du;
            }
        }
        const double cr = ref_cost<NS, NC>(x, ut, xf, Q, R, false);
        double cp[PPL > 0 ? PPL : 1];
#pragma unroll
        for (int q = 0; q < PPL; ++q) cp[q] = pair_cost_nd<NS>(sxs + (pp[q] & 255) * NS, sxs + ((pp[q] >> 8) & 255) * NS, pp[q] >> 16, radius);
        DPILQR_LDS_FENCE();
        post_costs(cr, cp, t & 1);
        double xn[NS];
        integrate<MODEL>(x, ut, D.dt, xn);
#pragma unroll
        for (int i = 0; i < NS; ++i) x[i] = xn[i];
        wave_sync<NW>();
    };
    if constexpr (PF == 1) {
        for (int t = 0; t < T; ++t) step(stg[0], t);
    } else {
        int t = 0;
        for (; t + 1 < T; t += 2) { step(stg[0], t); step(stg[1], t + 1); }
        if (t < T) step(stg[0], t);
    }
#ifdef DPILQR_PHASE_STAMPS
    if (g_stamp_buf && tid == 0) {
        g_stamp_buf[2 * slot] = w_wait;
        g_stamp_buf[2 * slot + 1] = __builtin_amdgcn_s_memtime() - w_t0;
    }
#endif
    if (active) {
        store_vec(Xw0 + (unsigned)(xw_off + T * n), x, NS);
        if (T > 0) store_vec(Uw0 + uw_off_at(T - 1), ut, NC);
    }
    {
        if (active) {
#pragma unroll
            for (int i = 0; i < NS; ++i) sxs[a * NS + i] = x[i];
        }
        wave_sync<NW>();
        if (a == 0 && T > 0) stage_cost(J, (T & 1) ^ 1);
        if constexpr (NS >= 6 || NW > 1) {
            int a2 = a;
            asm volatile("" : "+v"(a2));
            make_pairs(a2);
        }
        double Qf[NS * NS], uz[NC];
#pragma unroll
        for (int i = 0; i < NS * NS; ++i) Qf[i] = P.Qf[a * NS * NS + i];
#pragma unroll
        for (int c = 0; c < NC; ++c) uz[c] = 0.0;
        const double cr = ref_cost<NS, NC>(x, uz, xf, Qf, R, true);
        double cp[PPL > 0 ? PPL : 1];
#pragma unroll
        for (int q = 0; q < PPL; ++q) cp[q] = pair_cost_nd<NS>(sxs + (pp[q] & 255) * NS, sxs + ((pp[q] >> 8) & 255) * NS, pp[q] >> 16, radius);
        DPILQR_LDS_FENCE();
        post_costs(cr, cp, T & 1);
        wave_sync<NW>();
        if (a == 0) stage_cost(J, T & 1);
    }
    if constexpr (NS >= 6 || NW > 1) {
        int tid2 = tid;
        asm volatile("" : "+v"(tid2));
        if (active && a == 0) lds[W::oJ + tid2 / KA] = J;
    } else {
        if (active && a == 0) lds[W::oJ + g] = J;
    }
    asm volatile("s_waitcnt vmcnt(0)" ::: "memory");
    __builtin_amdgcn_fence(__ATOMIC_ACQ_REL, "workgroup");
    wave_sync<NW>();
    int* ctl = reinterpret_cast<int*>(lds + W::octl);
    if (tid == 0) ctl[0] = linesearch_decide(S, b, NG, lds + W::oJ);
    __builtin_amdgcn_fence(__ATOMIC_ACQ_REL, "workgroup");
    wave_sync<NW>();
    const int acc = ctl[0];
    if (acc < 0) return;
    const double* Xa = Xc + ((int64_t)slot * NG + acc) * (int64_t)(T + 1) * n;
    const double* Ua = Uc + ((int64_t)slot * NG + acc) * (int64_t)T * m;
    for (int e = tid; e < (T + 1) * n; e += NTH) Xb[e] = Xa[e];
    for (int e = tid; e < T * m; e += NTH) Ub[e] = Ua[e];
}

template <int MODEL, int KA>
struct WaveRolloutLds {
    static constexpr int NS = ModelDef<MODEL>::NS, n = KA * NS, NP = KA * (KA - 1) / 2, NP1 = NP > 0 ? NP : 1;
    static constexpr int IPW = 64 / KA;
    static constexpr int oxs = 0, ocr = oxs + IPW * n, ocp = ocr + IPW * KA, total = (ocp + IPW * NP1 + 1) & ~1;
};

template <int MODEL, int KA>
__global__ __launch_bounds__(256) void k_rollout_wave(dpilqr_batch_desc D, const double* __restrict__ x0,
                                                      const double* __restrict__ U, double* __restrict__ X,
                                                      double* __restrict__ Jout) {
    using W = WaveRolloutLds<MODEL, KA>;
    constexpr int NS = W::NS, NC = ModelDef<MODEL>::NC, n = W::n, m = KA * NC, NPAIRS = W::NP, NP1 = W::NP1, IPW = W::IPW;
    constexpr PairTable<KA> PT{};
    constexpr int PPL = (NPAIRS + KA - 1) / KA;
    const int sub = __builtin_amdgcn_readfirstlane((int)(threadIdx.x >> 6));
    const int tid = threadIdx.x & 63;
    const bool lane_on = tid < IPW * KA;
    const int w = lane_on ? tid / KA : 0, a = lane_on ? tid - (tid / KA) * KA : 0;
    const int64_t b_raw = ((int64_t)blockIdx.x * 4 + sub) * IPW + w;
    const bool active = lane_on && b_raw < D.B;
    const int b = (int)(b_raw < D.B ? b_raw : D.B - 1);
    const int T = D.T;
    extern __shared__ __attribute__((aligned(16))) double lds_all[];
    double* lds = lds_all + sub * W::total;
    double* sxs = lds + W::oxs + w * n;
    double* scr = lds + W::ocr + w * KA;
    double* scp = lds + W::ocp + w * NP1;
    const ItemParams P = item_params(D, b);
    double xf[NS], Q[NS * NS], R[NC * NC];
#pragma unroll
    for (int i = 0; i < NS; ++i) xf[i] = P.xf[a * NS + i];
#pragma unroll
    for (int i = 0; i < NS * NS; ++i) Q[i] = P.Q[a * NS * NS + i];
#pragma unroll
    for (int i = 0; i < NC * NC; ++i) R[i] = P.R[a * NC * NC + i];
    const double radius = P.radius;
    bool homog = true;
#pragma unroll
    for (int i = 1; i < KA; ++i) homog = homog && (P.n_dims[i] == P.n_dims[0]);
    int pi[PPL > 0 ? PPL : 1], pj[PPL > 0 ? PPL : 1], pnd[PPL > 0 ? PPL : 1];
#pragma unroll
    for (int q = 0; q < PPL; ++q) {
        const int p = min(a + q * KA, NP1 - 1);
        int ii = 0, jj = 0;
#pragma unroll
        for (int e = 0; e < NPAIRS; ++e)
            if (e == p) { ii = PT.i[e]; jj = PT.j[e]; }
        pi[q] = ii; pj[q] = jj;
        pnd[q] = homog ? 2 : min(P.n_dims[ii], P.n_dims[jj]);
    }
    const double* Ub = U + (int64_t)b * T * m + a * NC;
    double* Xw = X + (int64_t)b * (T + 1) * n + a * NS;
    auto store_vec = [&](double* p, const double* v, int len) {
        if ((len & 1) == 0) {
#pragma unroll
            for (int i = 0; i < len; i += 2) store_v2d_nt(p + i, v2d{v[i], v[i + 1]});
        } else {
#pragma unroll
            for (int i = 0; i < len; ++i) store_f64_nt(p + i, v[i]);
        }
    };
    auto stage_cost = [&](double& J) {
        double prox = 0.0, ref = 0.0;
#pragma unroll
        for (int p = 0; p < NPAIRS; ++p) prox += scp[p];
#pragma unroll
        for (int i = 0; i < KA; ++i) ref += scr[i];
        J += D.w_prox * prox + D.w_ref * ref;
    };
    double x[NS], u[NC], un[NC];
#pragma unroll
    for (int i = 0; i < NS; ++i) x[i] = x0[(int64_t)b * n + a * NS + i];
#pragma unroll
    for (int i = 0; i < NC; ++i) un[i] = (T > 0) ? Ub[i] : 0.0;
    double J = 0.0;
    for (int t = 0; t < T; ++t) {
        if (active) store_vec(Xw + (int64_t)t * n, x, NS);
#pragma unroll
        for (int i = 0; i < NC; ++i) u[i] = un[i];
        if (t + 1 < T) {
#pragma unroll
            for (int i = 0; i < NC; ++i) un[i] = Ub[(int64_t)(t + 1) * m + i];
        }
#pragma unroll
        for (int i = 0; i < NS; ++i) sxs[a * NS + i] = x[i];
        DPILQR_LDS_FENCE();
        if (a == 0 && t > 0) stage_cost(J);
        const double cr = ref_cost<NS, NC>(x, u, xf, Q, R, false);
        double cp[PPL > 0 ? PPL : 1];
#pragma unroll
        for (int q = 0; q < PPL; ++q) cp[q] = pair_cost_nd<NS>(sxs + pi[q] * NS, sxs + pj[q] * NS, pnd[q], radius);
        DPILQR_LDS_FENCE();
        scr[a] = cr;
#pragma unroll
        for (int q = 0; q < PPL; ++q)
            if (a + q * KA < NPAIRS) scp[a + q * KA] = cp[q];
        double xn[NS];
        integrate<MODEL>(x, u, D.dt, xn);
#pragma unroll
        for (int i = 0; i < NS; ++i) x[i] = xn[i];
    }
    if (active) store_vec(Xw + (int64_t)T * n, x, NS);
#pragma unroll
    for (int i = 0; i < NS; ++i) sxs[a * NS + i] = x[i];
    DPILQR_LDS_FENCE();
    if (a == 0 && T > 0) stage_cost(J);
    {
        double Qf[NS * NS], uz[NC];
#pragma unroll
        for (int i = 0; i < NS * NS; ++i) Qf[i] = P.Qf[a * NS * NS + i];
#pragma unroll
        for (int c = 0; c < NC; ++c) uz[c] = 0.0;
        const double cr = ref_cost<NS, NC>(x, uz, xf, Qf, R, true);
        double cp[PPL > 0 ? PPL : 1];
#pragma unroll
        for (int q = 0; q < PPL; ++q) cp[q] = pair_cost_nd<NS>(sxs + pi[q] * NS, sxs + pj[q] * NS, pnd[q], radius);
        DPILQR_LDS_FENCE();
        scr[a] = cr;
#pragma unroll
        for (int q = 0; q < PPL; ++q)
            if (a + q * KA < NPAIRS) scp[a + q * KA] = cp[q];
        DPILQR_LDS_FENCE();
        if (a == 0) stage_cost(J);
    }
    if (active && a == 0) Jout[b] = J;
}

}
```

### dpilqr_amd/csrc/launch.hpp

```cpp
#pragma once
#include <hip/hip_runtime.h>

#include <cstdint>
#include <cstdlib>

#include "dpilqr_hip.h"
#include "solve_state.hpp"

namespace dpilqr {

int32_t fail(int32_t code, const char* fmt, ...);
const char* last_error();

#define HIP_TRY(expr)                                                                                 \
    do {                                                                                              \
        hipError_t e_ = (expr);                                                                       \
        if (e_ != hipSuccess) return ::dpilqr::fail(DPILQR_EHIP, "%s failed: %s", #expr, hipGetErrorString(e_)); \
    } while (0)

constexpr int kMaxLds = 160 * 1024;

template <typename Kern>
inline int32_t allow_lds(Kern kern, size_t bytes) {
    if (bytes > (size_t)kMaxLds) return fail(DPILQR_EUNSUPPORTED, "needs %zu B of LDS per workgroup (> %d)", bytes, kMaxLds);
    if (bytes > 64 * 1024)
        HIP_TRY(hipFuncSetAttribute(reinterpret_cast<const void*>(kern), hipFuncAttributeMaxDynamicSharedMemorySize, (int)bytes));
    return DPILQR_OK;
}

#define DISPATCH_FAMILY_CASE(NS_, NC_, ...) case NS_: { constexpr int NS = NS_, NC = NC_; __VA_ARGS__ } break;
#define DISPATCH_FAMILY_CASES(ns, ...)                                                    \
    DISPATCH_FAMILY_CASE(3, 2, __VA_ARGS__)                                               \
    DISPATCH_FAMILY_CASE(4, 2, __VA_ARGS__)                                               \
    DISPATCH_FAMILY_CASE(6, 3, __VA_ARGS__)                                               \
    DISPATCH_FAMILY_CASE(12, 4, __VA_ARGS__)                                              \
    default: return ::dpilqr::fail(DPILQR_EINVAL, "unsupported per-agent state dim %d", (int)(ns));
#define DISPATCH_FAMILY(ns, BODY) switch (ns) { DISPATCH_FAMILY_CASES(ns, BODY) }
#define DISPATCH_FAMILY_ALL(ns, BODY) switch (ns) { DISPATCH_FAMILY_CASE(5, 2, BODY) DISPATCH_FAMILY_CASES(ns, BODY) }

int device_cus();

const char* route_env(const char* name);
inline bool route_flag(const char* name) { return route_env(name) != nullptr; }
inline int route_int(const char* name, int dflt) { const char* e = route_env(name); return (e && *e) ? atoi(e) : dflt; }

inline int hint_model(const dpilqr_batch_desc& D) { return (D.uniform_model & 0xff) - 1; }
inline int hint_n_dims(const dpilqr_batch_desc& D) { return ((D.uniform_model >> 8) & 0xff) - 1; }
inline bool hint_shared_weights(const dpilqr_batch_desc& D) { return ((D.uniform_model >> 16) & 1) != 0; }
inline bool hint_planar4(const dpilqr_batch_desc& D) { return ((D.uniform_model >> 17) & 1) != 0 || hint_model(D) == 0 || hint_model(D) == 3; }
inline bool fused_wavefront_sweep_applies(const dpilqr_batch_desc& D) {
    static const bool off = route_flag("DPILQR_NO_FUSED");
    return !off && hint_model(D) == 0 && hint_n_dims(D) == 2 && hint_shared_weights(D) && D.Q_bstride == 0 && D.R_bstride == 0 &&
           D.Qf_bstride == 0 && D.n_s == 4 && D.n_c == 2 && D.k <= 5;
}
inline bool fused_wavefront_general_applies(const dpilqr_batch_desc& D) {
    static const bool off = route_flag("DPILQR_NO_FUSED") || route_flag("DPILQR_NO_FUSED_GENERAL");
    return !off && hint_planar4(D) && hint_n_dims(D) == 2 && D.n_s == 4 && D.n_c == 2 && D.k <= 5;
}
inline bool fused_workgroup_sweep_applies(const dpilqr_batch_desc& D) {
    static const bool off = route_flag("DPILQR_NO_FUSED") || route_flag("DPILQR_NO_FUSED_WG");
    return !off && ((D.n_s == 4 && D.n_c == 2 && D.k >= 6 && D.k <= 15) || (D.n_s == 6 && D.n_c == 3 && D.k >= 2 && D.k <= 10));
}
inline bool fused_wavefront_inprod_applies(const dpilqr_batch_desc& D) {
    static const bool off = route_flag("DPILQR_NO_FUSED") || route_flag("DPILQR_NO_INPROD");
    static const bool no4 = route_flag("DPILQR_NO_INPROD4");
    if (off) return false;
    if (D.n_s == 4 && D.n_c == 2 && D.k <= 5 && !no4)
        return !fused_wavefront_sweep_applies(D) && !fused_wavefront_general_applies(D);
    return (D.n_s == 6 && D.n_c == 3 && D.k <= 4) || (D.n_s == 3 && D.n_c == 2 && D.k <= 6) || (D.n_s == 5 && D.n_c == 2 && D.k <= 4);
}
inline bool fused_sweep_applies(const dpilqr_batch_desc& D) {
    return fused_wavefront_sweep_applies(D) || fused_wavefront_general_applies(D) || fused_workgroup_sweep_applies(D) ||
           fused_wavefront_inprod_applies(D);
}
inline bool solve_prefers_records(const dpilqr_batch_desc& D) {
    static const bool off = route_flag("DPILQR_NO_WAVE_PREF");
    if (fused_wavefront_inprod_applies(D)) {
        static const bool rec = route_flag("DPILQR_INPROD_RECORDS");
        return rec || (!off && D.n_s == 5 && D.k <= 2);
    }
    return !off && ((D.n_s == 6 && D.n_c == 3 && (D.k == 2 || D.k == 3 || D.k == 4)) || (D.n_s == 4 && D.n_c == 2 && D.k == 6));
}

int32_t launch_make_tiles(const dpilqr_batch_desc& D, const double* X, const double* U, double* tiles,
                          const int32_t* items, const int32_t* n_items, int grid_items, bool sparse, bool dyn_only,
                          hipStream_t st);
int32_t tile_layout_host(int32_t n_x, int32_t n_u, int64_t offsets[7], int64_t row_strides[7], int64_t* stride);

extern thread_local int g_sweep_waves;
int32_t launch_riccati(int B, int T, int n, int m, const double* tiles, const double* mu, double* K, double* d,
                       int32_t* singular, const int32_t* items, const int32_t* n_items, int grid_items,
                       int gains_by_item, int block_ns, int block_nc, hipStream_t st);
int32_t launch_riccati_fused(const dpilqr_batch_desc& D, const double* X, const double* U, const double* mu, double* K,
                             double* d, int32_t* singular, const int32_t* items, const int32_t* n_items, int grid_items,
                             int gains_by_item, hipStream_t st);
int32_t set_stamp_buffer_riccati(void* device_buffer);

constexpr int sweep_waves(int grid_items, int max_wv, size_t lds_per_wave, bool tier12) {
    return (tier12 && grid_items > 2048 && max_wv >= 12 && lds_per_wave * 12 <= (size_t)kMaxLds) ? 12
           : (grid_items > 1024 && max_wv >= 8 && lds_per_wave * 8 <= (size_t)kMaxLds) ? 8 : 4;
}
constexpr int sweep_grid(int grid_items, int cus, int wv) {
    return grid_items <= cus ? grid_items : (grid_items + cus * wv - 1) / (cus * wv) * cus;
}
inline int sweep_max_waves() { static const int v = route_int("DPILQR_MFMA_WAVES", 12); return v; }
template <typename Kern, typename... Args>
int32_t launch_sweep_kernel(Kern kern, int wv, int threads, size_t lds, int grid_items, int cus, hipStream_t st, const Args&... args) {
    const int32_t rc = allow_lds(kern, lds);
    if (rc) return rc;
    hipLaunchKernelGGL(kern, dim3(sweep_grid(grid_items, cus, wv)), dim3(threads), lds, st, args...);
    HIP_TRY(hipGetLastError());
    g_sweep_waves = wv;
    return DPILQR_OK;
}
template <typename T> struct same_type { using type = T; };
template <typename Kern, typename... Args>
int32_t launch_wave_sweep(Kern k4, typename same_type<Kern>::type k8, typename same_type<Kern>::type k12, size_t lds_per_wave,
                          int grid_items, int cus, hipStream_t st, const Args&... args) {
    const int wv = sweep_waves(grid_items, sweep_max_waves(), lds_per_wave, k12 != nullptr);
    return launch_sweep_kernel(wv == 12 ? k12 : (wv == 8 ? k8 : k4), wv, 64 * wv, lds_per_wave * wv, grid_items, cus, st, args...);
}
int32_t launch_riccati_team(const dpilqr_batch_desc& D, const double* X, const double* U, const double* mu, double* K, double* d,
                            int32_t* singular, const int32_t* items, const int32_t* n_items, int grid_items, int gains_by_item,
                            hipStream_t st);

int32_t launch_riccati_inprod(const dpilqr_batch_desc& D, const double* X, const double* U, const double* mu, double* K, double* d,
                              int32_t* singular, const int32_t* items, const int32_t* n_items, int grid_items, int gains_by_item,
                              hipStream_t st);

int32_t launch_riccati_bike(const dpilqr_batch_desc& D, const double* X, const double* U, const double* mu, double* K, double* d,
                            int32_t* singular, const int32_t* items, const int32_t* n_items, int grid_items, int gains_by_item,
                            hipStream_t st);

int fused_sweep_tier(const dpilqr_batch_desc& D, int grid_items);
int32_t launch_cost_keys(const dpilqr_batch_desc& D, const double* X, const int32_t* list, const int32_t* count, int grid_items,
                         int min_live, int32_t* key, hipStream_t st);
int32_t launch_order_list(const int32_t* src, int32_t* dst, const int32_t* count, const int32_t* key, int T, int cus, int waves,
                          int order, int min_live, hipStream_t st);

int32_t launch_linesearch_team(const dpilqr_batch_desc& D, double* X, double* U, const double* K, const double* d,
                               const double* alphas, double* Xc, double* Uc, const SolveState& S, const int32_t* items,
                               const int32_t* n_items, int grid_items, hipStream_t st);

int32_t launch_forward(const dpilqr_batch_desc& D, int mode, const double* x0, double* X, double* U, const double* K,
                       const double* d, const double* alphas, int ngrp, double* Xc, double* Uc, double* Jc,
                       const SolveState& S, const int32_t* items, const int32_t* n_items, int grid_items,
                       hipStream_t st);
int32_t set_stamp_buffer_forward(void* device_buffer);
int32_t launch_model_op(int op, int32_t n, int32_t ns, const int32_t* model, const double* x, const double* u, double dt,
                        double* o1, double* o2, hipStream_t st);
int32_t launch_cost_eval(const dpilqr_batch_desc& D, int32_t n_pts, const double* x, const double* u, int32_t terminal,
                         double* cost, hipStream_t st);
int32_t launch_pairwise_graph(int32_t S, int32_t N, int32_t k, int32_t n_s, const double* X, const double* radius,
                              int32_t* adj, hipStream_t st);


int32_t launch_policy_rollout(const dpilqr_batch_desc& D, const double* X, const double* U, const double* K, int32_t n_samples,
                              const double* x0s, const double* W, const double* u_lim, double* Xs, double* Us, double* J,
                              double* min_sep, double* goal_dist, hipStream_t st);
int32_t launch_policy_rollout_dec(const dpilqr_batch_desc& D, const double* X, const double* U_ff, const double* Kc, int32_t kc_max,
                                  const uint64_t* nbr_bits, int32_t n_samples, const double* x0s, const double* W, const double* u_lim,
                                  double* Xs, double* Us, double* J, double* min_sep, double* goal_dist, hipStream_t st);

int32_t launch_policy_advance(const dpilqr_batch_desc& D, const double* X, const double* U, const double* K, int32_t kc_max,
                              const uint64_t* nbr_bits, int32_t h, const int32_t* scen, int32_t n_scen, int32_t L, int32_t n_d,
                              const double* W, const double* u_lim, double* x_cur, int32_t* n_done, double* X_exec, double* U_exec,
                              double* J_exec, double* min_sep, double* dist_left, double* U_next, double* X_next, hipStream_t st);

int32_t launch_policy_rollout_large(const dpilqr_batch_desc& D, const double* X, const double* U, const double* K, int32_t n_samples,
                                    const double* x0s, const double* W, const double* u_lim, double* Xs, double* Us, double* J,
                                    double* min_sep, double* goal_dist, hipStream_t st);

int32_t launch_policy_advance_large(const dpilqr_batch_desc& D, const double* X, const double* U, const double* K, int32_t h,
                                    const int32_t* scen, int32_t n_scen, int32_t L, int32_t n_d, const double* W, const double* u_lim,
                                    double* x_cur, int32_t* n_done, double* X_exec, double* U_exec, double* J_exec, double* min_sep,
                                    double* dist_left, double* U_next, double* X_next, hipStream_t st);

int32_t launch_rollout_wide(const dpilqr_batch_desc& D, const double* x0, const double* U, double* X, double* J, double* min_sep,
                            double* goal_dist, hipStream_t st);

int64_t riccati_big_scratch_elems(int n, int m);
int32_t launch_riccati_big_f64(const dpilqr_batch_desc& D, const double* X, const double* U, const double* mu, double* K,
                               double* d, int32_t* singular, const int32_t* items, const int32_t* n_items,
                               int grid_items, int gains_by_item, void* scratch, hipStream_t st);
int32_t launch_riccati_big_f32(const dpilqr_batch_desc& D, const float* X, const float* U, const double* mu, float* K,
                               float* d, int32_t* singular, const int32_t* items, const int32_t* n_items,
                               int grid_items, int gains_by_item, void* scratch, hipStream_t st);
int32_t launch_forward_big_f64(const dpilqr_batch_desc& D, int mode, const double* x0, double* X, double* U, const double* K,
                               const double* d, const double* alphas, int ngrp, double* Xc, double* Uc, double* Jc,
                               const SolveState& S, const int32_t* items, const int32_t* n_items, int grid_items,
                               hipStream_t st);
int32_t launch_forward_big_f32(const dpilqr_batch_desc& D, int mode, const float* x0, float* X, float* U, const float* K,
                               const float* d, const double* alphas, int ngrp, float* Xc, float* Uc, double* Jc,
                               const SolveState& S, const int32_t* items, const int32_t* n_items, int grid_items,
                               hipStream_t st);
inline bool uses_big_path(int n_x) {
    static const bool force = route_flag("DPILQR_FORCE_BIG");
    return force || n_x > 60;
}

}
```

### dpilqr_amd/csrc/tu_forward.hip

```cpp
#include <hip/hip_runtime.h>

#include <cstdlib>

#include "launch.hpp"
#include "forward.hpp"
#include "forward_wave.hpp"

namespace dpilqr {

static int forward_threads(int k, int ngrp) {
    const int t = ((k * ngrp + 63) / 64) * 64;
    return t;
}

static bool no_wave_ro() { static const bool v = route_flag("DPILQR_FORWARD_GENERIC"); return v; }

int32_t launch_forward(const dpilqr_batch_desc& D, int mode, const double* x0, double* X, double* U, const double* K,
                       const double* d, const double* alphas, int ngrp, double* Xc, double* Uc, double* Jc,
                       const SolveState& S, const int32_t* items, const int32_t* n_items, int grid_items,
                       hipStream_t st) {
    if (grid_items <= 0) return DPILQR_OK;
    const int n = D.k * D.n_s, m = D.k * D.n_c;
    int threads = forward_threads(D.k, mode == kModeRollout ? 1 : ngrp);
    if (threads > 256) return fail(DPILQR_EUNSUPPORTED, "k*n_alpha=%d exceeds the 256-thread workgroup of the forward pass", D.k * ngrp);
    const size_t lds_item = (forward_lds_bytes(n, m, D.k, ngrp) + 15) & ~(size_t)15;
    if (uses_big_path(n) || lds_item > (size_t)kMaxLds || (mode != kModeRollout && (m * n + threads - 1) / threads > kMaxStage))
        return launch_forward_big_f64(D, mode, x0, X, U, K, d, alphas, ngrp, Xc, Uc, Jc, S, items, n_items, grid_items, st);
    if (!no_wave_ro() && mode == kModeRollout && hint_model(D) >= 0 && !items) {
        const int model = hint_model(D);
#define DPILQR_TRY_RO(MODEL, KA)                                                                                    \
    if (model == MODEL && D.k == KA && model_ns(MODEL) == D.n_s && model_nc(MODEL) == D.n_c) {                      \
        using WR = WaveRolloutLds<MODEL, KA>;                                                                       \
        const int per_wg = 4 * WR::IPW;                                                                             \
        hipLaunchKernelGGL((k_rollout_wave<MODEL, KA>), dim3((grid_items + per_wg - 1) / per_wg), dim3(256),        \
                           sizeof(double) * WR::total * 4, st, D, x0, U, X, Jc);                                    \
        HIP_TRY(hipGetLastError());                                                                                 \
        return DPILQR_OK;                                                                                           \
    }
#define DPILQR_RO_10(MODEL) DPILQR_TRY_RO(MODEL, 1) DPILQR_TRY_RO(MODEL, 2) DPILQR_TRY_RO(MODEL, 3)                \
        DPILQR_TRY_RO(MODEL, 4) DPILQR_TRY_RO(MODEL, 5) DPILQR_TRY_RO(MODEL, 6) DPILQR_TRY_RO(MODEL, 7)             \
        DPILQR_TRY_RO(MODEL, 8) DPILQR_TRY_RO(MODEL, 9) DPILQR_TRY_RO(MODEL, 10)
#define DPILQR_RO_15(MODEL) DPILQR_RO_10(MODEL) DPILQR_TRY_RO(MODEL, 11) DPILQR_TRY_RO(MODEL, 12)                   \
        DPILQR_TRY_RO(MODEL, 13) DPILQR_TRY_RO(MODEL, 14) DPILQR_TRY_RO(MODEL, 15)
        DPILQR_RO_15(kDoubleInt4D)
        DPILQR_RO_15(kUnicycle4D)
        DPILQR_RO_10(kQuadcopter6D)
#define DPILQR_RO_6(MODEL) DPILQR_TRY_RO(MODEL, 1) DPILQR_TRY_RO(MODEL, 2) DPILQR_TRY_RO(MODEL, 3)                 \
        DPILQR_TRY_RO(MODEL, 4) DPILQR_TRY_RO(MODEL, 5) DPILQR_TRY_RO(MODEL, 6)
        DPILQR_RO_6(kDoubleInt6D)
        DPILQR_RO_6(kCar3D)
        DPILQR_RO_6(kBike5D)
        DPILQR_RO_6(kHuman6D)
        DPILQR_RO_6(kHumanLin6D)
        DPILQR_TRY_RO(kQuadcopter12D, 1) DPILQR_TRY_RO(kQuadcopter12D, 2) DPILQR_TRY_RO(kQuadcopter12D, 3)
        DPILQR_TRY_RO(kQuadcopter12D, 4) DPILQR_TRY_RO(kQuadcopter12D, 5)
#undef DPILQR_RO_6
#undef DPILQR_RO_15
#undef DPILQR_RO_10
#undef DPILQR_TRY_RO
    }
    static const bool no_wave = route_flag("DPILQR_FORWARD_GENERIC");
    if (!no_wave && mode == kModeLineSearch && hint_model(D) >= 0 && ngrp == DPILQR_N_ALPHA && items && n_items) {
        const int model = hint_model(D);
        {
            const int32_t rc_t = launch_linesearch_team(D, X, U, K, d, alphas, Xc, Uc, S, items, n_items, grid_items, st);
            if (rc_t != DPILQR_EUNSUPPORTED) return rc_t;
        }
#define DPILQR_TRY_WAVE(MODEL, KA)                                                                                  \
    if (model == MODEL && D.k == KA && model_ns(MODEL) == D.n_s && model_nc(MODEL) == D.n_c) {                      \
        using WF = WaveFwdLds<MODEL, KA>;                                                                           \
        const size_t lds_w = sizeof(double) * WF::total * WF::IPB;                                                  \
        int32_t rc_w = allow_lds(k_linesearch_wave<MODEL, KA>, lds_w);                                              \
        if (rc_w) return rc_w;                                                                                      \
        hipLaunchKernelGGL((k_linesearch_wave<MODEL, KA>), dim3((grid_items + WF::IPB - 1) / WF::IPB),              \
                           dim3(64 * WF::NW * WF::IPB), lds_w, st, D, X, U, K, d, alphas, Xc, Uc, S, items, n_items); \
        HIP_TRY(hipGetLastError());                                                                                 \
        return DPILQR_OK;                                                                                           \
    }
#define DPILQR_WAVE_10(MODEL) DPILQR_TRY_WAVE(MODEL, 1) DPILQR_TRY_WAVE(MODEL, 2) DPILQR_TRY_WAVE(MODEL, 3)        \
        DPILQR_TRY_WAVE(MODEL, 4) DPILQR_TRY_WAVE(MODEL, 5) DPILQR_TRY_WAVE(MODEL, 6) DPILQR_TRY_WAVE(MODEL, 7)     \
        DPILQR_TRY_WAVE(MODEL, 8) DPILQR_TRY_WAVE(MODEL, 9) DPILQR_TRY_WAVE(MODEL, 10)
#define DPILQR_WAVE_15(MODEL) DPILQR_WAVE_10(MODEL) DPILQR_TRY_WAVE(MODEL, 11) DPILQR_TRY_WAVE(MODEL, 12)           \
        DPILQR_TRY_WAVE(MODEL, 13) DPILQR_TRY_WAVE(MODEL, 14) DPILQR_TRY_WAVE(MODEL, 15)
        DPILQR_WAVE_15(kDoubleInt4D)
        DPILQR_WAVE_15(kUnicycle4D)
        DPILQR_WAVE_10(kQuadcopter6D)
#define DPILQR_WAVE_6(MODEL) DPILQR_TRY_WAVE(MODEL, 1) DPILQR_TRY_WAVE(MODEL, 2) DPILQR_TRY_WAVE(MODEL, 3)         \
        DPILQR_TRY_WAVE(MODEL, 4) DPILQR_TRY_WAVE(MODEL, 5) DPILQR_TRY_WAVE(MODEL, 6)
        DPILQR_WAVE_6(kDoubleInt6D)
        DPILQR_WAVE_6(kCar3D)
        DPILQR_WAVE_6(kBike5D)
        DPILQR_WAVE_6(kHuman6D)
        DPILQR_WAVE_6(kHumanLin6D)
        DPILQR_TRY_WAVE(kQuadcopter12D, 1) DPILQR_TRY_WAVE(kQuadcopter12D, 2) DPILQR_TRY_WAVE(kQuadcopter12D, 3)
        DPILQR_TRY_WAVE(kQuadcopter12D, 4)
#undef DPILQR_WAVE_6
#undef DPILQR_WAVE_15
#undef DPILQR_WAVE_10
#undef DPILQR_TRY_WAVE
    }
    static const bool no_pack = route_flag("DPILQR_FORWARD_NO_PACK");
    const int ipb = (!no_pack && threads == 64 && 4 * lds_item <= (size_t)kMaxLds) ? 4 : 1;
    const size_t lds = lds_item * ipb;
    threads *= ipb;
    DISPATCH_FAMILY_ALL(D.n_s, {
        int32_t rc = allow_lds(k_forward<double, NS, NC, false>, lds);
        if (rc) return rc;
        hipLaunchKernelGGL((k_forward<double, NS, NC, false>), dim3((grid_items + ipb - 1) / ipb), dim3(threads), lds, st, D, mode,
                           x0, X, U, K, d, alphas, ngrp, Xc, Uc, Jc, S, items, n_items, ipb, (int)(lds_item / sizeof(double)));
    })
    HIP_TRY(hipGetLastError());
    return DPILQR_OK;
}

int32_t set_stamp_buffer_forward(void* buf) {
    void* p = buf;
    HIP_TRY(hipMemcpyToSymbol(HIP_SYMBOL(g_stamp_buf), &p, sizeof(p)));
    return DPILQR_OK;
}

int32_t launch_model_op(int op, int32_t n, int32_t ns, const int32_t* model, const double* x, const double* u, double dt,
                        double* o1, double* o2, hipStream_t st) {
    const dim3 grid((n + 63) / 64), block(64);
    DISPATCH_FAMILY_ALL(ns, {
        if (op == 0) hipLaunchKernelGGL((k_model_op<NS, NC, 0>), grid, block, 0, st, n, model, x, u, dt, o1, o2);
        else if (op == 1) hipLaunchKernelGGL((k_model_op<NS, NC, 1>), grid, block, 0, st, n, model, x, u, dt, o1, o2);
        else hipLaunchKernelGGL((k_model_op<NS, NC, 2>), grid, block, 0, st, n, model, x, u, dt, o1, o2);
    })
    HIP_TRY(hipGetLastError());
    return DPILQR_OK;
}

int32_t launch_cost_eval(const dpilqr_batch_desc& D, int32_t n_pts, const double* x, const double* u, int32_t terminal,
                         double* cost, hipStream_t st) {
    const int64_t total = (int64_t)D.B * n_pts;
    const dim3 grid((unsigned)((total + 63) / 64)), block(64);
    DISPATCH_FAMILY_ALL(D.n_s, {
        hipLaunchKernelGGL((k_cost_eval<NS, NC>), grid, block, 0, st, D, n_pts, x, u, terminal, cost);
    })
    HIP_TRY(hipGetLastError());
    return DPILQR_OK;
}

int32_t launch_pairwise_graph(int32_t S, int32_t N, int32_t k, int32_t n_s, const double* X, const double* radius,
                              int32_t* adj, hipStream_t st) {
    HIP_TRY(hipMemsetAsync(adj, 0, sizeof(int32_t) * (size_t)S * k * k, st));
    const int64_t total = (int64_t)S * (k * (k - 1) / 2 + k);
    hipLaunchKernelGGL(k_pairwise_graph, dim3((unsigned)((total + 127) / 128)), dim3(128), 0, st, S, N, k, n_s, X, radius, adj);
    HIP_TRY(hipGetLastError());
    return DPILQR_OK;
}

}
```

### dpilqr_amd/csrc/tu_order.hip

```cpp
#include <hip/hip_runtime.h>

#define DPILQR_ADMIT_ORDER_KERNELS
#include "admit_order.hpp"
#include "launch.hpp"
#include "riccati_mfma.hpp"

namespace dpilqr {

int fused_sweep_tier(const dpilqr_batch_desc& D, int grid_items) {
    if (!fused_wavefront_sweep_applies(D) || grid_items <= kOrderMinLive) return 0;
    const int n = D.k * D.n_s, m = D.k * D.n_c;
#define DPILQR_TIER(NN, MM) \
    if (n == NN && m == MM) return sweep_waves(grid_items, sweep_max_waves(), sizeof(double) * MfmaCfg<NN, MM, true>::total, true);
    DPILQR_TIER(4, 2) DPILQR_TIER(8, 4) DPILQR_TIER(12, 6) DPILQR_TIER(16, 8) DPILQR_TIER(20, 10)
#undef DPILQR_TIER
    return 0;
}

int32_t launch_cost_keys(const dpilqr_batch_desc& D, const double* X, const int32_t* list, const int32_t* count, int grid_items,
                         int min_live, int32_t* key, hipStream_t st) {
    if (grid_items <= 0) return DPILQR_OK;
    hipLaunchKernelGGL(k_cost_keys, dim3((grid_items + 3) / 4), dim3(256), 0, st, X, D.radius, D.radius_bstride, list, count, D.B, D.T,
                       D.k, min_live, key);
    HIP_TRY(hipGetLastError());
    return DPILQR_OK;
}

int32_t launch_order_list(const int32_t* src, int32_t* dst, const int32_t* count, const int32_t* key, int T, int cus, int waves,
                          int order, int min_live, hipStream_t st) {
    hipLaunchKernelGGL(k_order_list, dim3(1), dim3(1024), 0, st, src, dst, count, key, T, cus, waves, order, min_live);
    HIP_TRY(hipGetLastError());
    return DPILQR_OK;
}

}
```

Measured before the change: 1.077 million subproblems/s.

## Fuse admission with cost ordering and compute near-keys inside line search

Merges the admit kernel and the order-list kernel into one single-workgroup admit_and_order kernel. The near-collision cost keys are now counted inside the double-integrator line-search kernel for the accepted alpha and stored per item, so the separate k_cost_keys pass that reread trajectories each iteration goes away. Keys come from the previous iteration's accepted trajectory, plus one initial key pass after rollout. This trades two launches and a full trajectory scan per iteration for extra work and a new kernel variant in line search, and the ordering keys may be one iteration stale.

```diff
diff --git a/dpilqr_amd/csrc/admit_order.hpp b/dpilqr_amd/csrc/admit_order.hpp
--- a/dpilqr_amd/csrc/admit_order.hpp
+++ b/dpilqr_amd/csrc/admit_order.hpp
@@ -4,8 +4,10 @@
 #if defined(__HIPCC__)
 #include <hip/hip_runtime.h>
 #define DPILQR_HD __host__ __device__
+#define DPILQR_UNROLL _Pragma("unroll")
 #else
 #define DPILQR_HD
+#define DPILQR_UNROLL
 #endif
 
 namespace dpilqr {
@@ -62,7 +64,137 @@
     return c < 0 ? 0 : (c > kOrderClasses - 1 ? kOrderClasses - 1 : c);
 }
 
+struct AdmitOrderArgs {
+    int32_t* list;
+    int32_t* out;
+    int32_t* count;
+    int32_t* next_count;
+    int32_t* admitted;
+    int B, window;
+    int32_t* mail;
+    int want_prefix;
+    int64_t* t_admit;
+    const int32_t* fault;
+    const int32_t* key;
+    int key_by_item;
+    int T, n_cus, waves, order, min_live;
+};
+
+struct SerialCtx {
+    int sh[2 * kOrderClasses + 1];
+    int64_t clock = 0;
+    int tid() const { return 0; }
+    int nthreads() const { return 1; }
+    void barrier() {}
+    int* scratch() { return sh; }
+    int atomic_add(int* p, int v) { const int old = *p; *p = old + v; return old; }
+    void atomic_min(int* p, int v) { if (v < *p) *p = v; }
+    void scan64(const int* hist, int* cursor) {
+        int run = 0;
+        for (int c = 0; c < kOrderClasses; ++c) { cursor[c] = run; run += hist[c]; }
+    }
+    int64_t now() const { return clock; }
+};
+
+template <class Ctx>
+DPILQR_HD inline void admit_and_order(const AdmitOrderArgs& a, Ctx& cx) {
+    int* hist = cx.scratch();
+    int* cursor = hist + kOrderClasses;
+    int* lowest = hist + 2 * kOrderClasses;
+    const int tid = cx.tid(), nt = cx.nthreads();
+    const int base = *a.count, first = *a.admitted;
+    const int room = a.window - base, left = a.B - first;
+    const int fit = left < room ? left : room;
+    const int n_new = fit > 0 ? fit : 0;
+    const int n = base + n_new;
+    const bool sort = a.out && a.order != kOrderOff && n > a.min_live;
+    if (tid == 0) *lowest = first;
+    for (int c = tid; c < kOrderClasses; c += nt) hist[c] = 0;
+    cx.barrier();
+    for (int i = tid; i < n_new; i += nt) a.list[base + i] = first + i;
+    if (a.t_admit && n_new > 0) {
+        const int64_t now = cx.now();
+        for (int i = tid; i < n_new; i += nt) a.t_admit[first + i] = now;
+    }
+    if (a.mail && a.want_prefix) {
+        int lo = first;
+        for (int i = tid; i < base; i += nt) { const int b = a.list[i]; lo = b < lo ? b : lo; }
+        if (lo < first) cx.atomic_min(lowest, lo);
+    }
+    auto item_at = [&](int i) { return i < base ? a.list[i] : first + (i - base); };
+    auto bin_of = [&](int i, int b) { return kOrderClasses - 1 - order_class(a.key[a.key_by_item ? b : i], a.T); };
+    constexpr int kAdmitHeld = 8;
+    const bool held = sort && n <= kAdmitHeld * nt;
+    int held_item[kAdmitHeld], held_bin[kAdmitHeld];
+    if (held) {
+        DPILQR_UNROLL
+        for (int q = 0; q < kAdmitHeld; ++q) { const int i = tid + q * nt; held_item[q] = i < n ? item_at(i) : -1; }
+        DPILQR_UNROLL
+        for (int q = 0; q < kAdmitHeld; ++q) held_bin[q] = held_item[q] >= 0 ? bin_of(tid + q * nt, held_item[q]) : 0;
+        DPILQR_UNROLL
+        for (int q = 0; q < kAdmitHeld; ++q)
+            if (held_item[q] >= 0) cx.atomic_add(&hist[held_bin[q]], 1);
+    } else if (sort) {
+        for (int i = tid; i < n; i += nt) cx.atomic_add(&hist[bin_of(i, item_at(i))], 1);
+    }
+    cx.barrier();
+    if (sort) {
+        cx.scan64(hist, cursor);
+        cx.barrier();
+        const SweepDeal deal(n, a.n_cus, a.waves);
+        auto place = [&](int b, int bin) {
+            const int rank = cx.atomic_add(&cursor[bin], 1);
+            const int pos = order_position(rank, deal, a.order);
+            if (pos >= 0 && pos < n) a.out[pos] = b;
+        };
+        if (held) {
+            DPILQR_UNROLL
+            for (int q = 0; q < kAdmitHeld; ++q)
+                if (held_item[q] >= 0) place(held_item[q], held_bin[q]);
+        } else {
+            for (int i = tid; i < n; i += nt) { const int b = item_at(i); place(b, bin_of(i, b)); }
+        }
+    } else if (a.out) {
+        for (int i = tid; i < n; i += nt) a.out[i] = item_at(i);
+    }
+    if (tid == 0) {
+        *a.count = n; *a.admitted = first + n_new; *a.next_count = 0;
+        if (a.mail) { a.mail[0] = n; a.mail[1] = first + n_new; a.mail[2] = a.want_prefix ? *lowest : 0; a.mail[3] = *a.fault; }
+    }
+}
+
+#if defined(__HIPCC__)
+struct WorkgroupCtx {
+    int* sh;
+    __device__ int tid() const { return (int)threadIdx.x; }
+    __device__ int nthreads() const { return (int)blockDim.x; }
+    __device__ void barrier() { __syncthreads(); }
+    __device__ int* scratch() { return sh; }
+    __device__ int atomic_add(int* p, int v) { return atomicAdd(p, v); }
+    __device__ void atomic_min(int* p, int v) { atomicMin(p, v); }
+    __device__ void scan64(const int* hist, int* cursor) {
+        static_assert(kOrderClasses == 64, "the prefix sums are one wavefront's, a bin per lane");
+        if (threadIdx.x < kOrderClasses) {
+            const int own = hist[threadIdx.x];
+            int run = own;
+            for (int off = 1; off < kOrderClasses; off <<= 1) {
+                const int below = __shfl_up(run, off);
+                if ((int)threadIdx.x >= off) run += below;
+            }
+            cursor[threadIdx.x] = run - own;
+        }
+    }
+    __device__ int64_t now() const { return (int64_t)__builtin_amdgcn_s_memrealtime(); }
+};
+#endif
+
 #if defined(__HIPCC__) && defined(DPILQR_ADMIT_ORDER_KERNELS)
+
+__global__ void __launch_bounds__(1024) k_admit_order(AdmitOrderArgs a) {
+    __shared__ int sh[2 * kOrderClasses + 1];
+    WorkgroupCtx cx{sh};
+    admit_and_order(a, cx);
+}
 
 constexpr int kKeyStagedAgents = 5;
 __global__ void __launch_bounds__(256) k_cost_keys(const double* __restrict__ X, const double* __restrict__ radius, int64_t radius_bstride,
diff --git a/dpilqr_amd/csrc/dpilqr_hip.hip b/dpilqr_amd/csrc/dpilqr_hip.hip
--- a/dpilqr_amd/csrc/dpilqr_hip.hip
+++ b/dpilqr_amd/csrc/dpilqr_hip.hip
@@ -105,31 +105,6 @@
     }
 }
 
-__global__ void k_admit(int32_t* list, int32_t* count, int32_t* next_count, int32_t* admitted, int B, int window,
-                        int32_t* mail, int want_prefix, int64_t* t_admit, const int32_t* fault) {
-    const int base = *count, first = *admitted;
-    const int n_new = min(B - first, window - base);
-    __shared__ int lowest;
-    if (threadIdx.x == 0) lowest = first;
-    __syncthreads();
-    for (int i = threadIdx.x; i < n_new; i += blockDim.x) list[base + i] = first + i;
-    if (t_admit && n_new > 0) {
-        const int64_t now = (int64_t)__builtin_amdgcn_s_memrealtime();
-        for (int i = threadIdx.x; i < n_new; i += blockDim.x) t_admit[first + i] = now;
-    }
-    if (mail && want_prefix) {
-        int lo = first;
-        for (int i = threadIdx.x; i < base; i += blockDim.x) lo = min(lo, list[i]);
-        for (int off = 32; off > 0; off >>= 1) lo = min(lo, __shfl_down(lo, off));
-        if ((threadIdx.x & 63) == 0) atomicMin(&lowest, lo);
-        __syncthreads();
-    }
-    if (threadIdx.x == 0) {
-        *count = base + n_new; *admitted = first + n_new; *next_count = 0;
-        if (mail) { mail[0] = base + n_new; mail[1] = first + n_new; mail[2] = want_prefix ? lowest : 0; mail[3] = *fault; }
-    }
-}
-
 __global__ void k_copy_f64(int n, const double* src, double* dst) {
     const int i = blockIdx.x * blockDim.x + threadIdx.x;
     if (i < n) dst[i] = src[i];
@@ -149,7 +124,7 @@
 };
 
 struct SolveWorkspace {
-    size_t tiles, K, d, Xc, Uc, mu, delta, J_star, J_last, alphas, singular, lists, counts, t_admit, total;
+    size_t tiles, K, d, Xc, Uc, mu, delta, J_star, J_last, alphas, singular, lists, counts, t_admit, near_key, total;
     SolveWorkspace(const dpilqr_batch_desc& D, int W, bool gains_in_ws, SolveShape sh) {
         const size_t B = D.B, n = (size_t)D.k * D.n_s, m = (size_t)D.k * D.n_c, T = D.T, Wn = W, e = sh.elem;
         const TileLayout L((int)n, (int)m);
@@ -170,6 +145,7 @@
         lists = o;    o = al(o + sizeof(int32_t) * 2 * Wn);
         counts = o;   o = al(o + sizeof(int32_t) * (kCountRing + 2));
         t_admit = o;  o = al(o + sizeof(int64_t) * B);
+        near_key = o; o = al(o + sizeof(int32_t) * B);
         total = o;
     }
 };
@@ -300,8 +276,9 @@
 template <> struct Passes<double> {
     static int32_t forward(const dpilqr_batch_desc& D, int mode, const double* x0, double* X, double* U, const double* K,
                            const double* d, const double* alphas, int ngrp, double* Xc, double* Uc, double* Jc,
-                           const SolveState& S, const int32_t* items, const int32_t* n_items, int grid, hipStream_t st) {
-        return launch_forward(D, mode, x0, X, U, K, d, alphas, ngrp, Xc, Uc, Jc, S, items, n_items, grid, st);
+                           const SolveState& S, const int32_t* items, const int32_t* n_items, int grid, hipStream_t st,
+                           int32_t* near_key = nullptr) {
+        return launch_forward(D, mode, x0, X, U, K, d, alphas, ngrp, Xc, Uc, Jc, S, items, n_items, grid, st, near_key);
     }
     static int32_t sweep_big(const dpilqr_batch_desc& D, const double* X, const double* U, const double* mu, double* K, double* d,
                              int32_t* sing, const int32_t* items, const int32_t* n_items, int grid, int by_item, void* scratch,
@@ -312,7 +289,8 @@
 template <> struct Passes<float> {
     static int32_t forward(const dpilqr_batch_desc& D, int mode, const float* x0, float* X, float* U, const float* K,
                            const float* d, const double* alphas, int ngrp, float* Xc, float* Uc, double* Jc,
-                           const SolveState& S, const int32_t* items, const int32_t* n_items, int grid, hipStream_t st) {
+                           const SolveState& S, const int32_t* items, const int32_t* n_items, int grid, hipStream_t st,
+                           int32_t* = nullptr) {
         return launch_forward_big_f32(D, mode, x0, X, U, K, d, alphas, ngrp, Xc, Uc, Jc, S, items, n_items, grid, st);
     }
     static int32_t sweep_big(const dpilqr_batch_desc& D, const float* X, const float* U, const double* mu, float* K, float* d,
@@ -400,6 +378,10 @@
     const bool fused = sh.fused;
     const bool static_part = !fused && !sh.big && !no_static && D.R_bstride == 0 &&
                              (um == kDoubleInt4D || um == kDoubleInt6D || um == kHumanLin6D);
+    static const int order_route = route_flag("DPILQR_NO_COST_ORDER") ? (int)kOrderOff : route_int("DPILQR_COST_ORDER", kDefaultCostOrder);
+    static const bool loop_keys = route_int("DPILQR_LOOP_KEYS", 1) != 0;
+    const int order = (sizeof(R) == 8 && fused && (order_route == kOrderSpread || order_route == kOrderGrouped)) ? order_route : (int)kOrderOff;
+    int32_t* const near_key = (order && loop_keys && fused_sweep_tier(D, Wn) > 0) ? reinterpret_cast<int32_t*>(ws + W.near_key) : nullptr;
     if (!resume) {
         double a[DPILQR_N_ALPHA];
         alpha_table(a);
@@ -412,6 +394,9 @@
                                 nullptr, D.B, st);
         if (rc) return bail(rc);
         prof.end(st);
+        if constexpr (sizeof(R) == 8) {
+            if (near_key && (rc = launch_cost_keys(D, X, nullptr, nullptr, D.B, -1, near_key, st))) return bail(rc);
+        }
         hipLaunchKernelGGL(k_copy_f64, dim3((D.B + 255) / 256), dim3(256), 0, st, D.B, S.J_star, S.J_last);
         if (n_lqr_iter > 0) {
             if (!fused && hipMemsetAsync(tiles, 0, W.K - W.tiles, st) != hipSuccess) return bail(fail(DPILQR_EHIP, "hipMemsetAsync failed"));
@@ -423,8 +408,6 @@
         }
     }
 
-    static const int order_route = route_flag("DPILQR_NO_COST_ORDER") ? (int)kOrderOff : route_int("DPILQR_COST_ORDER", kDefaultCostOrder);
-    const int order = (sizeof(R) == 8 && fused && (order_route == kOrderSpread || order_route == kOrderGrouped)) ? order_route : (int)kOrderOff;
     int32_t* keys = reinterpret_cast<int32_t*>(ws + W.Xc);
     int surv = 0;
     size_t n_iterations = 0;
@@ -434,15 +417,19 @@
         int32_t* cur_n = counts + (it % kCountRing);
         int32_t* nxt_n = counts + ((it + 1) % kCountRing);
         int32_t* mail = solver ? solver->dev + kMailWords * (it % kMailRing) : nullptr;
-        hipLaunchKernelGGL(k_admit, dim3(1), dim3(256), 0, st, cur, cur_n, nxt_n, admitted_dev, D.B, Wn, mail,
-                           (solver && solver->progress) ? 1 : 0, t_admit, S.fault);
-        if (solver) HIP_TRY(hipEventRecord(solver->ev[it % kMailRing], st));
         int32_t r = DPILQR_OK;
         const int order_waves = order ? fused_sweep_tier(D, upper) : 0;
+        AdmitOrderArgs ao{cur, nullptr, cur_n, nxt_n, admitted_dev, D.B, Wn, mail, (solver && solver->progress) ? 1 : 0, t_admit, S.fault,
+                          nullptr, 0, D.T, device_cus(), order_waves, order, kOrderMinLive};
+        if (order_waves > 0 && near_key) { ao.out = other; ao.key = near_key; ao.key_by_item = 1; }
+        if ((r = launch_admit_order(ao, st))) return r;
+        if (solver) HIP_TRY(hipEventRecord(solver->ev[it % kMailRing], st));
         if (order_waves > 0) {
             if constexpr (sizeof(R) == 8) {
-                if ((r = launch_cost_keys(D, X, cur, cur_n, upper, kOrderMinLive, keys, st))) return r;
-                if ((r = launch_order_list(cur, other, cur_n, keys, D.T, device_cus(), order_waves, order, kOrderMinLive, st))) return r;
+                if (!near_key) {
+                    if ((r = launch_cost_keys(D, X, cur, cur_n, upper, kOrderMinLive, keys, st))) return r;
+                    if ((r = launch_order_list(cur, other, cur_n, keys, D.T, device_cus(), order_waves, order, kOrderMinLive, st))) return r;
+                }
             }
             S.next_items = cur;
             cur = other;
@@ -475,7 +462,7 @@
         }
         prof.begin(2, it, st);
         if ((r = Passes<R>::forward(D, kModeLineSearch, nullptr, X, U, K, d, alphas, DPILQR_N_ALPHA, Xc, Uc, nullptr, S, cur, cur_n,
-                                    upper, st)))
+                                    upper, st, near_key)))
             return r;
         prof.end(st);
         return DPILQR_OK;
diff --git a/dpilqr_amd/csrc/forward_wave.hpp b/dpilqr_amd/csrc/forward_wave.hpp
--- a/dpilqr_amd/csrc/forward_wave.hpp
+++ b/dpilqr_amd/csrc/forward_wave.hpp
@@ -71,6 +71,23 @@
     const double m = fmin(0.0, sqrt(s) - radius);
     return m * m;
 }
+template <int NS>
+__device__ __forceinline__ double pair_cost_nd_near(const double* a, const double* b, int nd, double radius, bool& near) {
+    const double dx = a[0] - b[0], dy = a[1] - b[1];
+    double s = 0.0;
+    s += dx * dx;
+    s += dy * dy;
+    if (NS >= 3) {
+        const double dz = a[2] - b[2];
+        const double s3 = s + dz * dz;
+        s = (nd >= 3) ? s3 : s;
+    }
+    if (nd < 2) s = dx * dx;
+    near = !(s > radius * radius * (1.0 + 1e-12));
+    if (!near) return 0.0;
+    const double m = fmin(0.0, sqrt(s) - radius);
+    return m * m;
+}
 
 template <int MODEL, int KA>
 struct WaveFwdLds {
@@ -122,309 +139,26 @@
 }
 
 template <int MODEL, int KA>
+constexpr bool linesearch_keeps_keys = MODEL == kDoubleInt4D && KA <= 5;
+
+template <int MODEL, int KA>
 __global__ __launch_bounds__((64 * WaveFwdLds<MODEL, KA>::NW * WaveFwdLds<MODEL, KA>::IPB), (WaveFwdLds<MODEL, KA>::OCC)) void k_linesearch_wave(
     dpilqr_batch_desc D, double* X, double* U, const double* __restrict__ K, const double* __restrict__ d,
     const double* __restrict__ alphas, double* Xc, double* Uc, SolveState S, const int32_t* __restrict__ items,
     const int32_t* __restrict__ n_items) {
-    using W = WaveFwdLds<MODEL, KA>;
-    constexpr int NS = W::NS, NC = W::NC, n = W::n, m = W::m, mn = m * n, NPAIRS = W::NP, NP1 = W::NP1;
-    constexpr int NG = DPILQR_N_ALPHA;
-    constexpr int NW = W::NW, NTH = 64 * NW;
-    constexpr int PPL = (NPAIRS + KA - 1) / KA;
-    constexpr int KV = (mn / 2 + NTH - 1) / NTH;
-
-    const int sub = NW == 1 ? __builtin_amdgcn_readfirstlane((int)(threadIdx.x >> 6)) : 0;
-    const int tid = NW == 1 ? (int)(threadIdx.x & 63) : (int)threadIdx.x;
-    const int slot = blockIdx.x * W::IPB + sub;
-    if (slot >= *n_items) return;
-    const int b = items[slot];
-    const int T = D.T;
-    extern __shared__ __attribute__((aligned(16))) double lds_all[];
-    double* lds = lds_all + sub * W::total;
-    double* Xb = X + (int64_t)b * (T + 1) * n;
-    double* Ub = U + (int64_t)b * T * m;
-    if (S.singular && S.singular[b]) {
-        if (tid == 0) retire_without_gains(S, b);
-        return;
-    }
-    const int64_t gslot = S.gains_by_item ? b : slot;
-    const double* Kb = K + gslot * T * mn;
-    const double* db = d + gslot * T * m;
-    const bool active = tid < KA * NG;
-    const int g = active ? tid / KA : 0, a = active ? tid - (tid / KA) * KA : 0;
-    const double alpha = alphas[g];
-    double* const Xw0 = Xc + (int64_t)slot * NG * (int64_t)(T + 1) * n;
-    double* const Uw0 = Uc + (int64_t)slot * NG * (int64_t)T * m;
-    int xw_off = g * (T + 1) * n + a * NS;
-    asm volatile("" : "+v"(xw_off));
-    auto uw_off_at = [&](int t_) {
-        int g_ = g;
-        asm volatile("" : "+v"(g_));
-        return (unsigned)(g_ * (T * m) + a * NC + t_ * m);
-    };
-
-    const ItemParams P = item_params(D, b);
-    constexpr bool CL = W::CONST_LDS;
-    double xf_r[CL ? 1 : NS], Q_r[CL ? 1 : NS * NS], R_r[CL ? 1 : NC * NC];
-    const double* xf = xf_r; const double* Q = Q_r; const double* R = R_r;
-    if constexpr (CL) {
-        for (int e = tid; e < KA * NS * NS; e += NTH) lds[W::oQ + e] = P.Q[e];
-        for (int e = tid; e < KA * NC * NC; e += NTH) lds[W::oR + e] = P.R[e];
-        for (int e = tid; e < n; e += NTH) lds[W::oXf + e] = P.xf[e];
-        xf = lds + W::oXf + a * NS; Q = lds + W::oQ + a * NS * NS; R = lds + W::oR + a * NC * NC;
-    } else {
-#pragma unroll
-        for (int i = 0; i < NS; ++i) xf_r[i] = P.xf[a * NS + i];
-#pragma unroll
-        for (int i = 0; i < NS * NS; ++i) Q_r[i] = P.Q[a * NS * NS + i];
-#pragma unroll
-        for (int i = 0; i < NC * NC; ++i) R_r[i] = P.R[a * NC * NC + i];
-    }
-    const double radius = P.radius;
-    bool homog = true;
-#pragma unroll
-    for (int i = 1; i < KA; ++i) homog = homog && (P.n_dims[i] == P.n_dims[0]);
-    int pp[PPL > 0 ? PPL : 1];
-    auto make_pairs = [&](int a_) {
-#pragma unroll
-        for (int q = 0; q < PPL; ++q) {
-            const int p = min(a_ + q * KA, NP1 - 1);
-            int ii = 0, rem = p;
-            while (rem >= KA - 1 - ii) { rem -= KA - 1 - ii; ++ii; }
-            const int jj = ii + 1 + rem;
-            pp[q] = ii | (jj << 8) | ((homog ? 2 : min(P.n_dims[ii], P.n_dims[jj])) << 16);
-        }
-    };
-    make_pairs(a);
-
-    double* sK = lds + W::oK;
-    double* sd = lds + W::od;
-    double* sdx = lds + W::odx + g * W::LDG;
-    double* sxs = lds + W::oxs + g * W::LDG;
-    double* scr0 = lds + W::ocr + g * KA;
-    double* scp0 = lds + W::ocp + g * NP1;
-
-    struct Stage { v2d stK[KV]; double std_, u[NC], xold[NS]; };
-    constexpr int PF = W::PF;
-    Stage stg[PF];
-    double x[NS];
-    auto fetch = [&](Stage& sg, int t) {
-        const unsigned ko = (unsigned)(t * mn), xo = (unsigned)(t * n + a * NS), uo = (unsigned)(t * m + a * NC);
-#ifdef DPILQR_LS_K_FIRST
-#pragma unroll
-        for (int q = 0; q < KV; ++q) {
-            const int e = min(tid + NTH * q, mn / 2 - 1);
-            sg.stK[q] = *reinterpret_cast<const v2d*>(Kb + (ko + 2u * (unsigned)e));
-        }
-#endif
-#pragma unroll
-        for (int i = 0; i < NS; ++i) sg.xold[i] = Xb[xo + (unsigned)i];
-#pragma unroll
-        for (int i = 0; i < NC; ++i) sg.u[i] = Ub[uo + (unsigned)i];
-        sg.std_ = db[(unsigned)(t * m + min(tid, m - 1))];
-#ifndef DPILQR_LS_K_FIRST
-#pragma unroll
-        for (int q = 0; q < KV; ++q) {
-            const int e = min(tid + NTH * q, mn / 2 - 1);
-            sg.stK[q] = *reinterpret_cast<const v2d*>(Kb + (ko + 2u * (unsigned)e));
-        }
-#endif
-    };
-    auto store_vec = [&](double* p, const double* v, int len) {
-        if ((len & 1) == 0) {
-#pragma unroll
-            for (int i = 0; i < len; i += 2) store_v2d_nt(p + i, v2d{v[i], v[i + 1]});
-        } else {
-#pragma unroll
-            for (int i = 0; i < len; ++i) store_f64_nt(p + i, v[i]);
-        }
-    };
-    auto stage_cost = [&](double& J, int par) {
-        const double* scp = scp0 + par * NG * NP1;
-        const double* scr = scr0 + par * NG * KA;
-        double prox = 0.0, ref = 0.0;
-        if constexpr (NPAIRS > 32) {
-            constexpr int CH = 8;
-#pragma unroll 1
-            for (int p0 = 0; p0 < NPAIRS; p0 += CH) {
-                double v[CH];
-#pragma unroll
-                for (int q = 0; q < CH; ++q) v[q] = scp[min(p0 + q, NP1 - 1)];
-#pragma unroll
-                for (int q = 0; q < CH; ++q) prox = (p0 + q < NPAIRS) ? prox + v[q] : prox;
-            }
-        } else {
-#pragma unroll
-            for (int p = 0; p < NPAIRS; ++p) prox += scp[p];
-        }
-#pragma unroll
-        for (int i = 0; i < KA; ++i) ref += scr[i];
-        J += D.w_prox * prox + D.w_ref * ref;
-    };
-    auto post_costs = [&](double cr, const double* cp, int par) {
-        if (active) {
-            scr0[par * NG * KA + a] = cr;
-#pragma unroll
-            for (int q = 0; q < PPL; ++q)
-                if (a + q * KA < NPAIRS) scp0[par * NG * NP1 + a + q * KA] = cp[q];
-        }
-    };
-
-#pragma unroll
-    for (int i = 0; i < NS; ++i) x[i] = Xb[a * NS + i];
-#pragma unroll
-    for (int s = 0; s < PF; ++s)
-        if (s < T) fetch(stg[s], s);
-    double J = 0.0;
-    double ut[NC];
-#pragma unroll
-    for (int i = 0; i < NC; ++i) ut[i] = 0.0;
-
-#ifdef DPILQR_PHASE_STAMPS
-    unsigned long long w_wait = 0, w_t0 = __builtin_amdgcn_s_memtime();
-#endif
-    auto step = [&](Stage& sg, int t) {
-        v2d (&stK)[KV] = sg.stK;
-        double& std_ = sg.std_;
-        double (&u)[NC] = sg.u;
-        double (&xold)[NS] = sg.xold;
-#ifdef DPILQR_PHASE_STAMPS
-        {
-            const unsigned long long a0 = __builtin_amdgcn_s_memtime();
-            asm volatile("s_waitcnt vmcnt(0)" ::: "memory");
-            w_wait += __builtin_amdgcn_s_memtime() - a0;
-        }
-#endif
-#pragma unroll
-        for (int q = 0; q < KV; ++q) {
-            int tid_o = tid;
-            if constexpr (W::KGAP > 0) asm volatile("" : "+v"(tid_o));
-            const int e = min(tid_o + NTH * q, mn / 2 - 1);
-            *reinterpret_cast<v2d*>(sK + 2 * e + (W::KGAP > 0 ? ((2 * e) / W::KBLK) * W::KGAP : 0)) = stK[q];
-        }
-        if (tid < m) sd[tid] = std_;
-        if (active) {
-            store_vec(Xw0 + (unsigned)(xw_off + t * n), x, NS);
-            if (t > 0) store_vec(Uw0 + uw_off_at(t - 1), ut, NC);
-        }
-#pragma unroll
-        for (int i = 0; i < NC; ++i) ut[i] = u[i];
-        if (active) {
-#pragma unroll
-            for (int i = 0; i < NS; ++i) {
-                sdx[a * NS + i] = x[i] - xold[i];
-                sxs[a * NS + i] = x[i];
-            }
-        }
-        wave_sync<NW>();
-        if (t + PF < T) fetch(sg, t + PF);
-        if (a == 0 && t > 0) stage_cost(J, (t & 1) ^ 1);
-        DPILQR_LDS_FENCE();
-        {
-            double sum[NC];
-#pragma unroll
-            for (int c = 0; c < NC; ++c) sum[c] = 0.0;
-            const double* rows = sK + a * (W::KBLK + W::KGAP);
-            if (n % 2 == 0) {
-#pragma unroll 5
-                for (int j = 0; j < n; j += 2) {
-                    const v2d dx2 = *reinterpret_cast<const v2d*>(lds + W::odx + g * W::LDG + j);
-#pragma unroll
-                    for (int c = 0; c < NC; ++c) {
-                        const v2d kr = *reinterpret_cast<const v2d*>(rows + c * n + j);
-                        sum[c] += kr.x * dx2.x;
-                        sum[c] += kr.y * dx2.y;
-                    }
-                }
-            } else {
-#pragma unroll
-                for (int j = 0; j < n; ++j) {
-                    const double dxj = lds[W::odx + g * W::LDG + j];
-#pragma unroll
-                    for (int c = 0; c < NC; ++c) sum[c] += rows[c * n + j] * dxj;
-                }
-            }
-#pragma unroll
-            for (int c = 0; c < NC; ++c) {
-                const double du = sum[c] + alpha * sd[a * NC + c];
-                ut[c] = ut[c] + du;
-            }
-        }
-        const double cr = ref_cost<NS, NC>(x, ut, xf, Q, R, false);
-        double cp[PPL > 0 ? PPL : 1];
-#pragma unroll
-        for (int q = 0; q < PPL; ++q) cp[q] = pair_cost_nd<NS>(sxs + (pp[q] & 255) * NS, sxs + ((pp[q] >> 8) & 255) * NS, pp[q] >> 16, radius);
-        DPILQR_LDS_FENCE();
-        post_costs(cr, cp, t & 1);
-        double xn[NS];
-        integrate<MODEL>(x, ut, D.dt, xn);
-#pragma unroll
-        for (int i = 0; i < NS; ++i) x[i] = xn[i];
-        wave_sync<NW>();
-    };
-    if constexpr (PF == 1) {
-        for (int t = 0; t < T; ++t) step(stg[0], t);
-    } else {
-        int t = 0;
-        for (; t + 1 < T; t += 2) { step(stg[0], t); step(stg[1], t + 1); }
-        if (t < T) step(stg[0], t);
-    }
-#ifdef DPILQR_PHASE_STAMPS
-    if (g_stamp_buf && tid == 0) {
-        g_stamp_buf[2 * slot] = w_wait;
-        g_stamp_buf[2 * slot + 1] = __builtin_amdgcn_s_memtime() - w_t0;
-    }
-#endif
-    if (active) {
-        store_vec(Xw0 + (unsigned)(xw_off + T * n), x, NS);
-        if (T > 0) store_vec(Uw0 + uw_off_at(T - 1), ut, NC);
-    }
-    {
-        if (active) {
-#pragma unroll
-            for (int i = 0; i < NS; ++i) sxs[a * NS + i] = x[i];
-        }
-        wave_sync<NW>();
-        if (a == 0 && T > 0) stage_cost(J, (T & 1) ^ 1);
-        if constexpr (NS >= 6 || NW > 1) {
-            int a2 = a;
-            asm volatile("" : "+v"(a2));
-            make_pairs(a2);
-        }
-        double Qf[NS * NS], uz[NC];
-#pragma unroll
-        for (int i = 0; i < NS * NS; ++i) Qf[i] = P.Qf[a * NS * NS + i];
-#pragma unroll
-        for (int c = 0; c < NC; ++c) uz[c] = 0.0;
-        const double cr = ref_cost<NS, NC>(x, uz, xf, Qf, R, true);
-        double cp[PPL > 0 ? PPL : 1];
-#pragma unroll
-        for (int q = 0; q < PPL; ++q) cp[q] = pair_cost_nd<NS>(sxs + (pp[q] & 255) * NS, sxs + ((pp[q] >> 8) & 255) * NS, pp[q] >> 16, radius);
-        DPILQR_LDS_FENCE();
-        post_costs(cr, cp, T & 1);
-        wave_sync<NW>();
-        if (a == 0) stage_cost(J, T & 1);
-    }
-    if constexpr (NS >= 6 || NW > 1) {
-        int tid2 = tid;
-        asm volatile("" : "+v"(tid2));
-        if (active && a == 0) lds[W::oJ + tid2 / KA] = J;
-    } else {
-        if (active && a == 0) lds[W::oJ + g] = J;
-    }
-    asm volatile("s_waitcnt vmcnt(0)" ::: "memory");
-    __builtin_amdgcn_fence(__ATOMIC_ACQ_REL, "workgroup");
-    wave_sync<NW>();
-    int* ctl = reinterpret_cast<int*>(lds + W::octl);
-    if (tid == 0) ctl[0] = linesearch_decide(S, b, NG, lds + W::oJ);
-    __builtin_amdgcn_fence(__ATOMIC_ACQ_REL, "workgroup");
-    wave_sync<NW>();
-    const int acc = ctl[0];
-    if (acc < 0) return;
-    const double* Xa = Xc + ((int64_t)slot * NG + acc) * (int64_t)(T + 1) * n;
-    const double* Ua = Uc + ((int64_t)slot * NG + acc) * (int64_t)T * m;
-    for (int e = tid; e < (T + 1) * n; e += NTH) Xb[e] = Xa[e];
-    for (int e = tid; e < T * m; e += NTH) Ub[e] = Ua[e];
+#define DPILQR_LS_KEYS 0
+#include "forward_wave_body.inc"
+#undef DPILQR_LS_KEYS
+}
+
+template <int MODEL, int KA>
+__global__ __launch_bounds__((64 * WaveFwdLds<MODEL, KA>::NW * WaveFwdLds<MODEL, KA>::IPB), (WaveFwdLds<MODEL, KA>::OCC)) void k_linesearch_wave_keys(
+    dpilqr_batch_desc D, double* X, double* U, const double* __restrict__ K, const double* __restrict__ d,
+    const double* __restrict__ alphas, double* Xc, double* Uc, SolveState S, const int32_t* __restrict__ items,
+    const int32_t* __restrict__ n_items, int32_t* near_key) {
+#define DPILQR_LS_KEYS 1
+#include "forward_wave_body.inc"
+#undef DPILQR_LS_KEYS
 }
 
 template <int MODEL, int KA>
diff --git a/dpilqr_amd/csrc/forward_wave_body.inc b/dpilqr_amd/csrc/forward_wave_body.inc
--- /dev/null
+++ b/dpilqr_amd/csrc/forward_wave_body.inc
@@ -0,0 +1,338 @@
+    using W = WaveFwdLds<MODEL, KA>;
+#if DPILQR_LS_KEYS
+    static_assert(W::NW == 1 && W::NS == 4, "the key counter is one wavefront's ballot over planar four-state agents");
+#endif
+    constexpr int NS = W::NS, NC = W::NC, n = W::n, m = W::m, mn = m * n, NPAIRS = W::NP, NP1 = W::NP1;
+    constexpr int NG = DPILQR_N_ALPHA;
+    constexpr int NW = W::NW, NTH = 64 * NW;
+    constexpr int PPL = (NPAIRS + KA - 1) / KA;
+    constexpr int KV = (mn / 2 + NTH - 1) / NTH;
+
+    const int sub = NW == 1 ? __builtin_amdgcn_readfirstlane((int)(threadIdx.x >> 6)) : 0;
+    const int tid = NW == 1 ? (int)(threadIdx.x & 63) : (int)threadIdx.x;
+    const int slot = blockIdx.x * W::IPB + sub;
+    if (slot >= *n_items) return;
+    const int b = items[slot];
+    const int T = D.T;
+    extern __shared__ __attribute__((aligned(16))) double lds_all[];
+    double* lds = lds_all + sub * W::total;
+    double* Xb = X + (int64_t)b * (T + 1) * n;
+    double* Ub = U + (int64_t)b * T * m;
+    if (S.singular && S.singular[b]) {
+        if (tid == 0) retire_without_gains(S, b);
+        return;
+    }
+    const int64_t gslot = S.gains_by_item ? b : slot;
+    const double* Kb = K + gslot * T * mn;
+    const double* db = d + gslot * T * m;
+    const bool active = tid < KA * NG;
+    const int g = active ? tid / KA : 0, a = active ? tid - (tid / KA) * KA : 0;
+    const double alpha = alphas[g];
+    double* const Xw0 = Xc + (int64_t)slot * NG * (int64_t)(T + 1) * n;
+    double* const Uw0 = Uc + (int64_t)slot * NG * (int64_t)T * m;
+    int xw_off = g * (T + 1) * n + a * NS;
+    asm volatile("" : "+v"(xw_off));
+    auto uw_off_at = [&](int t_) {
+        int g_ = g;
+        asm volatile("" : "+v"(g_));
+        return (unsigned)(g_ * (T * m) + a * NC + t_ * m);
+    };
+
+    const ItemParams P = item_params(D, b);
+    constexpr bool CL = W::CONST_LDS;
+    double xf_r[CL ? 1 : NS], Q_r[CL ? 1 : NS * NS], R_r[CL ? 1 : NC * NC];
+    const double* xf = xf_r; const double* Q = Q_r; const double* R = R_r;
+    if constexpr (CL) {
+        for (int e = tid; e < KA * NS * NS; e += NTH) lds[W::oQ + e] = P.Q[e];
+        for (int e = tid; e < KA * NC * NC; e += NTH) lds[W::oR + e] = P.R[e];
+        for (int e = tid; e < n; e += NTH) lds[W::oXf + e] = P.xf[e];
+        xf = lds + W::oXf + a * NS; Q = lds + W::oQ + a * NS * NS; R = lds + W::oR + a * NC * NC;
+    } else {
+#pragma unroll
+        for (int i = 0; i < NS; ++i) xf_r[i] = P.xf[a * NS + i];
+#pragma unroll
+        for (int i = 0; i < NS * NS; ++i) Q_r[i] = P.Q[a * NS * NS + i];
+#pragma unroll
+        for (int i = 0; i < NC * NC; ++i) R_r[i] = P.R[a * NC * NC + i];
+    }
+    const double radius = P.radius;
+    bool homog = true;
+#pragma unroll
+    for (int i = 1; i < KA; ++i) homog = homog && (P.n_dims[i] == P.n_dims[0]);
+    int pp[PPL > 0 ? PPL : 1];
+    auto make_pairs = [&](int a_) {
+#pragma unroll
+        for (int q = 0; q < PPL; ++q) {
+            const int p = min(a_ + q * KA, NP1 - 1);
+            int ii = 0, rem = p;
+            while (rem >= KA - 1 - ii) { rem -= KA - 1 - ii; ++ii; }
+            const int jj = ii + 1 + rem;
+            pp[q] = ii | (jj << 8) | ((homog ? 2 : min(P.n_dims[ii], P.n_dims[jj])) << 16);
+        }
+    };
+    make_pairs(a);
+
+    double* sK = lds + W::oK;
+    double* sd = lds + W::od;
+    double* sdx = lds + W::odx + g * W::LDG;
+    double* sxs = lds + W::oxs + g * W::LDG;
+    double* scr0 = lds + W::ocr + g * KA;
+    double* scp0 = lds + W::ocp + g * NP1;
+
+    struct Stage { v2d stK[KV]; double std_, u[NC], xold[NS]; };
+    constexpr int PF = W::PF;
+    Stage stg[PF];
+    double x[NS];
+    auto fetch = [&](Stage& sg, int t) {
+        const unsigned ko = (unsigned)(t * mn), xo = (unsigned)(t * n + a * NS), uo = (unsigned)(t * m + a * NC);
+#ifdef DPILQR_LS_K_FIRST
+#pragma unroll
+        for (int q = 0; q < KV; ++q) {
+            const int e = min(tid + NTH * q, mn / 2 - 1);
+            sg.stK[q] = *reinterpret_cast<const v2d*>(Kb + (ko + 2u * (unsigned)e));
+        }
+#endif
+#pragma unroll
+        for (int i = 0; i < NS; ++i) sg.xold[i] = Xb[xo + (unsigned)i];
+#pragma unroll
+        for (int i = 0; i < NC; ++i) sg.u[i] = Ub[uo + (unsigned)i];
+        sg.std_ = db[(unsigned)(t * m + min(tid, m - 1))];
+#ifndef DPILQR_LS_K_FIRST
+#pragma unroll
+        for (int q = 0; q < KV; ++q) {
+            const int e = min(tid + NTH * q, mn / 2 - 1);
+            sg.stK[q] = *reinterpret_cast<const v2d*>(Kb + (ko + 2u * (unsigned)e));
+        }
+#endif
+    };
+    auto store_vec = [&](double* p, const double* v, int len) {
+        if ((len & 1) == 0) {
+#pragma unroll
+            for (int i = 0; i < len; i += 2) store_v2d_nt(p + i, v2d{v[i], v[i + 1]});
+        } else {
+#pragma unroll
+            for (int i = 0; i < len; ++i) store_f64_nt(p + i, v[i]);
+        }
+    };
+    auto stage_cost = [&](double& J, int par) {
+        const double* scp = scp0 + par * NG * NP1;
+        const double* scr = scr0 + par * NG * KA;
+        double prox = 0.0, ref = 0.0;
+        if constexpr (NPAIRS > 32) {
+            constexpr int CH = 8;
+#pragma unroll 1
+            for (int p0 = 0; p0 < NPAIRS; p0 += CH) {
+                double v[CH];
+#pragma unroll
+                for (int q = 0; q < CH; ++q) v[q] = scp[min(p0 + q, NP1 - 1)];
+#pragma unroll
+                for (int q = 0; q < CH; ++q) prox = (p0 + q < NPAIRS) ? prox + v[q] : prox;
+            }
+        } else {
+#pragma unroll
+            for (int p = 0; p < NPAIRS; ++p) prox += scp[p];
+        }
+#pragma unroll
+        for (int i = 0; i < KA; ++i) ref += scr[i];
+        J += D.w_prox * prox + D.w_ref * ref;
+    };
+    auto post_costs = [&](double cr, const double* cp, int par) {
+        if (active) {
+            scr0[par * NG * KA + a] = cr;
+#pragma unroll
+            for (int q = 0; q < PPL; ++q)
+                if (a + q * KA < NPAIRS) scp0[par * NG * NP1 + a + q * KA] = cp[q];
+        }
+    };
+
+#pragma unroll
+    for (int i = 0; i < NS; ++i) x[i] = Xb[a * NS + i];
+#pragma unroll
+    for (int s = 0; s < PF; ++s)
+        if (s < T) fetch(stg[s], s);
+    double J = 0.0;
+    double ut[NC];
+#pragma unroll
+    for (int i = 0; i < NC; ++i) ut[i] = 0.0;
+#if DPILQR_LS_KEYS
+    int n_near = 0;
+    auto count_near = [&](bool near) {
+        const unsigned long long mask = __builtin_amdgcn_ballot_w64(near);
+        n_near += ((unsigned)(mask >> (g * KA)) & ((1u << KA) - 1u)) != 0u ? 1 : 0;
+    };
+#endif
+
+#ifdef DPILQR_PHASE_STAMPS
+    unsigned long long w_wait = 0, w_t0 = __builtin_amdgcn_s_memtime();
+#endif
+    auto step = [&](Stage& sg, int t) {
+        v2d (&stK)[KV] = sg.stK;
+        double& std_ = sg.std_;
+        double (&u)[NC] = sg.u;
+        double (&xold)[NS] = sg.xold;
+#ifdef DPILQR_PHASE_STAMPS
+        {
+            const unsigned long long a0 = __builtin_amdgcn_s_memtime();
+            asm volatile("s_waitcnt vmcnt(0)" ::: "memory");
+            w_wait += __builtin_amdgcn_s_memtime() - a0;
+        }
+#endif
+#pragma unroll
+        for (int q = 0; q < KV; ++q) {
+            int tid_o = tid;
+            if constexpr (W::KGAP > 0) asm volatile("" : "+v"(tid_o));
+            const int e = min(tid_o + NTH * q, mn / 2 - 1);
+            *reinterpret_cast<v2d*>(sK + 2 * e + (W::KGAP > 0 ? ((2 * e) / W::KBLK) * W::KGAP : 0)) = stK[q];
+        }
+        if (tid < m) sd[tid] = std_;
+        if (active) {
+            store_vec(Xw0 + (unsigned)(xw_off + t * n), x, NS);
+            if (t > 0) store_vec(Uw0 + uw_off_at(t - 1), ut, NC);
+        }
+#pragma unroll
+        for (int i = 0; i < NC; ++i) ut[i] = u[i];
+        if (active) {
+#pragma unroll
+            for (int i = 0; i < NS; ++i) {
+                sdx[a * NS + i] = x[i] - xold[i];
+                sxs[a * NS + i] = x[i];
+            }
+        }
+        wave_sync<NW>();
+        if (t + PF < T) fetch(sg, t + PF);
+        if (a == 0 && t > 0) stage_cost(J, (t & 1) ^ 1);
+        DPILQR_LDS_FENCE();
+        {
+            double sum[NC];
+#pragma unroll
+            for (int c = 0; c < NC; ++c) sum[c] = 0.0;
+            const double* rows = sK + a * (W::KBLK + W::KGAP);
+            if (n % 2 == 0) {
+#pragma unroll 5
+                for (int j = 0; j < n; j += 2) {
+                    const v2d dx2 = *reinterpret_cast<const v2d*>(lds + W::odx + g * W::LDG + j);
+#pragma unroll
+                    for (int c = 0; c < NC; ++c) {
+                        const v2d kr = *reinterpret_cast<const v2d*>(rows + c * n + j);
+                        sum[c] += kr.x * dx2.x;
+                        sum[c] += kr.y * dx2.y;
+                    }
+                }
+            } else {
+#pragma unroll
+                for (int j = 0; j < n; ++j) {
+                    const double dxj = lds[W::odx + g * W::LDG + j];
+#pragma unroll
+                    for (int c = 0; c < NC; ++c) sum[c] += rows[c * n + j] * dxj;
+                }
+            }
+#pragma unroll
+            for (int c = 0; c < NC; ++c) {
+                const double du = sum[c] + alpha * sd[a * NC + c];
+                ut[c] = ut[c] + du;
+            }
+        }
+        const double cr = ref_cost<NS, NC>(x, ut, xf, Q, R, false);
+        double cp[PPL > 0 ? PPL : 1];
+#if DPILQR_LS_KEYS
+        {
+            bool near = false;
+#pragma unroll
+            for (int q = 0; q < PPL; ++q) {
+                bool near_q;
+                cp[q] = pair_cost_nd_near<NS>(sxs + (pp[q] & 255) * NS, sxs + ((pp[q] >> 8) & 255) * NS, pp[q] >> 16, radius, near_q);
+                near = near || near_q;
+            }
+            count_near(near);
+        }
+#else
+#pragma unroll
+        for (int q = 0; q < PPL; ++q) cp[q] = pair_cost_nd<NS>(sxs + (pp[q] & 255) * NS, sxs + ((pp[q] >> 8) & 255) * NS, pp[q] >> 16, radius);
+#endif
+        DPILQR_LDS_FENCE();
+        post_costs(cr, cp, t & 1);
+        double xn[NS];
+        integrate<MODEL>(x, ut, D.dt, xn);
+#pragma unroll
+        for (int i = 0; i < NS; ++i) x[i] = xn[i];
+        wave_sync<NW>();
+    };
+    if constexpr (PF == 1) {
+        for (int t = 0; t < T; ++t) step(stg[0], t);
+    } else {
+        int t = 0;
+        for (; t + 1 < T; t += 2) { step(stg[0], t); step(stg[1], t + 1); }
+        if (t < T) step(stg[0], t);
+    }
+#ifdef DPILQR_PHASE_STAMPS
+    if (g_stamp_buf && tid == 0) {
+        g_stamp_buf[2 * slot] = w_wait;
+        g_stamp_buf[2 * slot + 1] = __builtin_amdgcn_s_memtime() - w_t0;
+    }
+#endif
+    if (active) {
+        store_vec(Xw0 + (unsigned)(xw_off + T * n), x, NS);
+        if (T > 0) store_vec(Uw0 + uw_off_at(T - 1), ut, NC);
+    }
+    {
+        if (active) {
+#pragma unroll
+            for (int i = 0; i < NS; ++i) sxs[a * NS + i] = x[i];
+        }
+        wave_sync<NW>();
+        if (a == 0 && T > 0) stage_cost(J, (T & 1) ^ 1);
+        if constexpr (NS >= 6 || NW > 1) {
+            int a2 = a;
+            asm volatile("" : "+v"(a2));
+            make_pairs(a2);
+        }
+        double Qf[NS * NS], uz[NC];
+#pragma unroll
+        for (int i = 0; i < NS * NS; ++i) Qf[i] = P.Qf[a * NS * NS + i];
+#pragma unroll
+        for (int c = 0; c < NC; ++c) uz[c] = 0.0;
+        const double cr = ref_cost<NS, NC>(x, uz, xf, Qf, R, true);
+        double cp[PPL > 0 ? PPL : 1];
+#if DPILQR_LS_KEYS
+        {
+            bool near = false;
+#pragma unroll
+            for (int q = 0; q < PPL; ++q) {
+                bool near_q;
+                cp[q] = pair_cost_nd_near<NS>(sxs + (pp[q] & 255) * NS, sxs + ((pp[q] >> 8) & 255) * NS, pp[q] >> 16, radius, near_q);
+                near = near || near_q;
+            }
+            count_near(near);
+        }
+#else
+#pragma unroll
+        for (int q = 0; q < PPL; ++q) cp[q] = pair_cost_nd<NS>(sxs + (pp[q] & 255) * NS, sxs + ((pp[q] >> 8) & 255) * NS, pp[q] >> 16, radius);
+#endif
+        DPILQR_LDS_FENCE();
+        post_costs(cr, cp, T & 1);
+        wave_sync<NW>();
+        if (a == 0) stage_cost(J, T & 1);
+    }
+    if constexpr (NS >= 6 || NW > 1) {
+        int tid2 = tid;
+        asm volatile("" : "+v"(tid2));
+        if (active && a == 0) lds[W::oJ + tid2 / KA] = J;
+    } else {
+        if (active && a == 0) lds[W::oJ + g] = J;
+    }
+    asm volatile("s_waitcnt vmcnt(0)" ::: "memory");
+    __builtin_amdgcn_fence(__ATOMIC_ACQ_REL, "workgroup");
+    wave_sync<NW>();
+    int* ctl = reinterpret_cast<int*>(lds + W::octl);
+    if (tid == 0) ctl[0] = linesearch_decide(S, b, NG, lds + W::oJ);
+    __builtin_amdgcn_fence(__ATOMIC_ACQ_REL, "workgroup");
+    wave_sync<NW>();
+    const int acc = ctl[0];
+    if (acc < 0) return;
+#if DPILQR_LS_KEYS
+    if (tid == acc * KA) near_key[b] = n_near;
+#endif
+    const double* Xa = Xc + ((int64_t)slot * NG + acc) * (int64_t)(T + 1) * n;
+    const double* Ua = Uc + ((int64_t)slot * NG + acc) * (int64_t)T * m;
+    for (int e = tid; e < (T + 1) * n; e += NTH) Xb[e] = Xa[e];
+    for (int e = tid; e < T * m; e += NTH) Ub[e] = Ua[e];
diff --git a/dpilqr_amd/csrc/launch.hpp b/dpilqr_amd/csrc/launch.hpp
--- a/dpilqr_amd/csrc/launch.hpp
+++ b/dpilqr_amd/csrc/launch.hpp
@@ -137,6 +137,8 @@
                          int min_live, int32_t* key, hipStream_t st);
 int32_t launch_order_list(const int32_t* src, int32_t* dst, const int32_t* count, const int32_t* key, int T, int cus, int waves,
                           int order, int min_live, hipStream_t st);
+struct AdmitOrderArgs;
+int32_t launch_admit_order(const AdmitOrderArgs& a, hipStream_t st);
 
 int32_t launch_linesearch_team(const dpilqr_batch_desc& D, double* X, double* U, const double* K, const double* d,
                                const double* alphas, double* Xc, double* Uc, const SolveState& S, const int32_t* items,
@@ -145,7 +147,7 @@
 int32_t launch_forward(const dpilqr_batch_desc& D, int mode, const double* x0, double* X, double* U, const double* K,
                        const double* d, const double* alphas, int ngrp, double* Xc, double* Uc, double* Jc,
                        const SolveState& S, const int32_t* items, const int32_t* n_items, int grid_items,
-                       hipStream_t st);
+                       hipStream_t st, int32_t* near_key = nullptr);
 int32_t set_stamp_buffer_forward(void* device_buffer);
 int32_t launch_model_op(int op, int32_t n, int32_t ns, const int32_t* model, const double* x, const double* u, double dt,
                         double* o1, double* o2, hipStream_t st);
diff --git a/dpilqr_amd/csrc/tu_forward.hip b/dpilqr_amd/csrc/tu_forward.hip
--- a/dpilqr_amd/csrc/tu_forward.hip
+++ b/dpilqr_amd/csrc/tu_forward.hip
@@ -15,10 +15,34 @@
 
 static bool no_wave_ro() { static const bool v = route_flag("DPILQR_FORWARD_GENERIC"); return v; }
 
+template <int MODEL, int KA>
+static int32_t launch_linesearch_wave(const dpilqr_batch_desc& D, double* X, double* U, const double* K, const double* d,
+                                      const double* alphas, double* Xc, double* Uc, const SolveState& S, const int32_t* items,
+                                      const int32_t* n_items, int grid_items, hipStream_t st, int32_t* near_key) {
+    using WF = WaveFwdLds<MODEL, KA>;
+    const size_t lds_w = sizeof(double) * WF::total * WF::IPB;
+    const dim3 grid((grid_items + WF::IPB - 1) / WF::IPB), block(64 * WF::NW * WF::IPB);
+    if constexpr (linesearch_keeps_keys<MODEL, KA>) {
+        if (near_key) {
+            const int32_t rc_k = allow_lds(k_linesearch_wave_keys<MODEL, KA>, lds_w);
+            if (rc_k) return rc_k;
+            hipLaunchKernelGGL((k_linesearch_wave_keys<MODEL, KA>), grid, block, lds_w, st, D, X, U, K, d, alphas, Xc, Uc, S, items, n_items,
+                               near_key);
+            HIP_TRY(hipGetLastError());
+            return DPILQR_OK;
+        }
+    }
+    const int32_t rc_w = allow_lds(k_linesearch_wave<MODEL, KA>, lds_w);
+    if (rc_w) return rc_w;
+    hipLaunchKernelGGL((k_linesearch_wave<MODEL, KA>), grid, block, lds_w, st, D, X, U, K, d, alphas, Xc, Uc, S, items, n_items);
+    HIP_TRY(hipGetLastError());
+    return DPILQR_OK;
+}
+
 int32_t launch_forward(const dpilqr_batch_desc& D, int mode, const double* x0, double* X, double* U, const double* K,
                        const double* d, const double* alphas, int ngrp, double* Xc, double* Uc, double* Jc,
                        const SolveState& S, const int32_t* items, const int32_t* n_items, int grid_items,
-                       hipStream_t st) {
+                       hipStream_t st, int32_t* near_key) {
     if (grid_items <= 0) return DPILQR_OK;
     const int n = D.k * D.n_s, m = D.k * D.n_c;
     int threads = forward_threads(D.k, mode == kModeRollout ? 1 : ngrp);
@@ -67,16 +91,8 @@
             if (rc_t != DPILQR_EUNSUPPORTED) return rc_t;
         }
 #define DPILQR_TRY_WAVE(MODEL, KA)                                                                                  \
-    if (model == MODEL && D.k == KA && model_ns(MODEL) == D.n_s && model_nc(MODEL) == D.n_c) {                      \
-        using WF = WaveFwdLds<MODEL, KA>;                                                                           \
-        const size_t lds_w = sizeof(double) * WF::total * WF::IPB;                                                  \
-        int32_t rc_w = allow_lds(k_linesearch_wave<MODEL, KA>, lds_w);                                              \
-        if (rc_w) return rc_w;                                                                                      \
-        hipLaunchKernelGGL((k_linesearch_wave<MODEL, KA>), dim3((grid_items + WF::IPB - 1) / WF::IPB),              \
-                           dim3(64 * WF::NW * WF::IPB), lds_w, st, D, X, U, K, d, alphas, Xc, Uc, S, items, n_items); \
-        HIP_TRY(hipGetLastError());                                                                                 \
-        return DPILQR_OK;                                                                                           \
-    }
+    if (model == MODEL && D.k == KA && model_ns(MODEL) == D.n_s && model_nc(MODEL) == D.n_c)                        \
+        return launch_linesearch_wave<MODEL, KA>(D, X, U, K, d, alphas, Xc, Uc, S, items, n_items, grid_items, st, near_key);
 #define DPILQR_WAVE_10(MODEL) DPILQR_TRY_WAVE(MODEL, 1) DPILQR_TRY_WAVE(MODEL, 2) DPILQR_TRY_WAVE(MODEL, 3)        \
         DPILQR_TRY_WAVE(MODEL, 4) DPILQR_TRY_WAVE(MODEL, 5) DPILQR_TRY_WAVE(MODEL, 6) DPILQR_TRY_WAVE(MODEL, 7)     \
         DPILQR_TRY_WAVE(MODEL, 8) DPILQR_TRY_WAVE(MODEL, 9) DPILQR_TRY_WAVE(MODEL, 10)
diff --git a/dpilqr_amd/csrc/tu_order.hip b/dpilqr_amd/csrc/tu_order.hip
--- a/dpilqr_amd/csrc/tu_order.hip
+++ b/dpilqr_amd/csrc/tu_order.hip
@@ -26,6 +26,12 @@
     return DPILQR_OK;
 }
 
+int32_t launch_admit_order(const AdmitOrderArgs& a, hipStream_t st) {
+    hipLaunchKernelGGL(k_admit_order, dim3(1), dim3(a.out ? 1024 : 256), 0, st, a);
+    HIP_TRY(hipGetLastError());
+    return DPILQR_OK;
+}
+
 int32_t launch_order_list(const int32_t* src, int32_t* dst, const int32_t* count, const int32_t* key, int T, int cus, int waves,
                           int order, int min_live, hipStream_t st) {
     hipLaunchKernelGGL(k_order_list, dim3(1), dim3(1024), 0, st, src, dst, count, key, T, cus, waves, order, min_live);
```

Result: no change. 1.073 million subproblems/s, median of 2 (-0.4%).
